# BBCG/epialleleR

Hardware: AMD Instinct MI355X
Metric: Mreads/s generateCytosineReport (150 bp PE) (higher is better)
Workload: dtype u8

## Files before the change

### epialleler_amd/csrc/common.hpp

```cpp
#pragma once
#include <hip/hip_runtime.h>
#include <stddef.h>
#include <stdint.h>
#include <string>
#include <map>
#include <memory>
#include <vector>
#include "../../include/epihip.h"

namespace epi {

void set_error(const char *fmt, ...);
int fail(int code, const char *fmt, ...);

#define EPI_HIP(expr)                                                              \
  do {                                                                             \
    hipError_t _e = (expr);                                                        \
    if (_e != hipSuccess)                                                          \
      return ::epi::fail(_e == hipErrorOutOfMemory ? EPI_ERR_NOMEM : EPI_ERR_HIP,  \
                         "%s failed: %s (%s:%d)", #expr, hipGetErrorName(_e), __FILE__, __LINE__); \
  } while (0)

#define EPI_TRY(expr) do { int _rc = (expr); if (_rc != EPI_OK) return _rc; } while (0)
constexpr int EPI_RETRY_POOL = -77;

#ifndef EPI_CX_TILE
#define EPI_CX_TILE 1024
#endif
constexpr int kTile = EPI_CX_TILE;
constexpr int kMhlTile = 512;
constexpr int kCxPlanes = 16;
constexpr int64_t kPosBias = 1LL << 31;

enum { SLOT_DOT = 0, SLOT_OTHER = 1, SLOT_H = 2, SLOT_h = 3, SLOT_X = 4, SLOT_x = 5, SLOT_Z = 6, SLOT_z = 7, SLOT_SKIP = 8 };

struct Tile {
  int64_t pos0;
  int32_t rname;
  int32_t row_lo, row_hi;
  int32_t slot;
};

struct Scalars {
  uint32_t ntiles;
  uint32_t cursor;
  uint32_t rows;
  uint32_t heavy_count;
  uint32_t deep_count;
  uint32_t fold_cursor;
  uint32_t unused6[2];
  uint32_t heavy_max;
  uint32_t unused9[3];
  uint32_t rec_max[2];
  uint32_t max_h;
  uint32_t pat_total;
};
static_assert(offsetof(Scalars, ntiles) == 0 && offsetof(Scalars, cursor) == 4 && offsetof(Scalars, rows) == 8 &&
              offsetof(Scalars, heavy_count) == 12 && offsetof(Scalars, deep_count) == 16 && offsetof(Scalars, fold_cursor) == 20 &&
              offsetof(Scalars, heavy_max) == 32 && offsetof(Scalars, rec_max) == 48 && offsetof(Scalars, max_h) == 56 &&
              offsetof(Scalars, pat_total) == 60 && sizeof(Scalars) == 64, "Scalars layout");

struct DevBuf {
  void *p = nullptr;
  size_t cap = 0;
  int ensure(size_t bytes);
  void release();
  template <class T> T *as() const { return reinterpret_cast<T *>(p); }
};

struct ProfEntry { double ms = 0; int64_t n = 0; };

struct ClassLut { uint32_t lo0, lo1, hi0, hi1; };

inline ClassLut lut16_xor_form(const ClassLut &d) {
  uint8_t D[16], L[8], H[8];
  const uint32_t w[4] = {d.lo0, d.lo1, d.hi0, d.hi1};
  for (int c = 0; c < 16; c++) D[c] = (uint8_t)(w[c >> 2] >> (8 * (c & 3)));
  auto S = [](uint8_t x) { return (uint8_t)((x & 0x80u) ? 0xFFu : 0x00u); };
  L[4] = D[4]; H[4] = D[12];
  for (int j = 5; j < 8; j++) { L[j] = (uint8_t)~D[j]; H[j] = (uint8_t)~D[8 + j]; }
  L[2] = D[2] ^ S(H[5]); L[3] = D[3] ^ S(H[7]); H[2] = D[10] ^ S(L[5]); H[3] = D[11] ^ S(L[7]);
  L[1] = D[1] ^ S(H[3]); H[1] = D[9] ^ S(L[3]);
  L[0] = D[0] ^ S(H[1]); H[0] = D[8] ^ S(L[1]);
  auto pack = [](const uint8_t *b) { return (uint32_t)b[0] | ((uint32_t)b[1] << 8) | ((uint32_t)b[2] << 16) | ((uint32_t)b[3] << 24); };
  ClassLut x;
  x.lo0 = pack(L); x.lo1 = pack(L + 4); x.hi0 = pack(H); x.hi1 = pack(H + 4);
  return x;
}
struct ThrParams {
  uint32_t min_n_ctx;
  double min_ctx_meth_frac, max_ooctx_meth_frac;
};
bool make_field_lut(const char *const cls[4], ClassLut *out);

}

struct epi_engine {
  int device = 0;
  hipStream_t stream = nullptr;
  hipStream_t copy_stream = nullptr;
  void *pinned[2] = {nullptr, nullptr};
  size_t pinned_bytes = 0;
  hipEvent_t pinned_done[2] = {nullptr, nullptr};
  hipStream_t aux_stream = nullptr;
  void *dev_stage[2] = {nullptr, nullptr};
  size_t dev_stage_bytes = 0;
  hipEvent_t up_done[2] = {nullptr, nullptr}, stage_free[2] = {nullptr, nullptr};
  int32_t *h_scalars = nullptr;
};

namespace epi {
struct RowStats {
  int32_t max_len;
  int32_t unsorted;
  int32_t bad_strand;
  int32_t bad_len;
  int32_t deep;
  uint32_t len_hist[14];
};
constexpr int kLenBinCount = 14;
constexpr int kLenBins[kLenBinCount] = {12, 16, 20, 24, 32, 40, 48, 64, 80, 96, 128, 160, 192, 0x7FFFFFFF};
}

struct epi_shard_plan;

namespace epi {
enum ReportKind {
  KIND_NONE = 0,
  KIND_CX = 1,
  KIND_MHL = 2,
  KIND_CX_SHARED = 3,
  KIND_MHL_SHARED = 4,
  KIND_MHLF_SHARED = 5,
  KIND_HET = 6,
  KIND_LINK = 7,
  KIND_HETCMP = 8,
};
}

struct epi_batch {
  epi_engine *eng = nullptr;
  int64_t n = 0, nbytes = 0;
  const uint8_t *xm = nullptr;
  const int64_t *off = nullptr;
  const int32_t *len = nullptr;
  const int32_t *rname = nullptr, *strand = nullptr, *start = nullptr;
  bool owns = false;
  int congruent = 0;
  bool cols_owned = false;
  epi::DevBuf own_xm, own_off, own_len, own_rname, own_strand, own_start;

  epi::DevBuf stats;
  bool stats_queued = false, stats_host = false;
  hipEvent_t stats_done = nullptr;
  epi::RowStats h_stats = {};
  epi::DevBuf scan_tmp;
  epi::DevBuf tiles, tile_nrow, tile_base, tile_out;
  epi::DevBuf pool_key, pool_a, pool_b, pool_c, pool_d, pool_e, pool_f;
  epi::DevBuf misc;
  epi::DevBuf mhl_m, mhl_h, mhl_blk, mhl_cont, mhl_cur;
  size_t mhl_rec_cap = 0;
  epi::DevBuf heavy_list, heavy_slab, heavy_sums;
  epi::DevBuf deep_list;
  epi::DevBuf diag;
  size_t pool_cap = 0;
  uint32_t cx_slot_cg = 0, cx_slot_wide = 0;
  uint32_t mhl_slot = 0, mhl_last_slot = 0, mhl_last_ovf = 0;
  uint32_t mhlf_slot = 0;
  bool mhlf_prefer_wide = false;
  uint32_t mhlf_prefer_wide_H = 0;
  bool mhlf_prefer_fold = false;
  epi::DevBuf mhlf_fold_slab;
  bool mhl_shared_fused = false;
  uint32_t cx_last_slot = 0, cx_last_ovf = 0;
  epi::DevBuf cx_prev_off, cx_prev_cnt;
  uint32_t cx_prev_key = 0;
  int32_t cx_prev_T = 0, cx_prev_nt = 0;
  int64_t cx_prev_nrow = 0;
  bool cx_defer = false, cx_deferred = false;
  uint32_t cx_def_heavy_done = 0;
  int32_t cx_noheavy_T = 0, cx_noheavy_rows = 0;
  int cx_last_np = 0;
  uint32_t cx_last_ctx_of_plane = 0;
  epi::DevBuf pass_tmp;
  epi::DevBuf host_io;
  epi::DevBuf bf_flag;
  int64_t patm_groups = 0, patm_pairs = 0, patm_scratch = 0;
  int64_t pats_groups = 0, pats_pairs = 0, pats_fallback = 0;
  epi::DevBuf mhl_keep_tab;
  int32_t mhl_keep_len = -1;
  double mhl_keep_oo = 0.0;
  epi::DevBuf thr_tab;
  int32_t thr_tab_len = -1;
  epi::ThrParams thr_tab_prm = {0, 0.0, 0.0};
  size_t pool_cap2 = 0;
  epi::DevBuf het_cx, het_rank, het_flag, het_key, het_sctx, het_counts, het_out, het_scal;
  int64_t het_nsite = 0, het_max_span = 0;
  int32_t het_k = 0;
  uint32_t het_min_reads = 1;
  epi::DevBuf link_back, link_blen, link_bmean, link_bflag, link_bout;
  int32_t link_D = 0;
  uint32_t link_min_reads = 1;
  int64_t link_max_dist = 0, link_nblock = 0;
  bool link_blocks = false;
  epi::DevBuf cmp_cx, cmp_counts_b;

  epi::ReportKind last_kind = epi::KIND_NONE;
  int64_t last_nrow = 0;
  int32_t last_ntiles = 0;
  int32_t tile_hint_T[4] = {0, 0, 0, 0};
  int32_t tile_hint_nt[4] = {0, 0, 0, 0};
  int32_t tile_hint_lmax[4] = {0, 0, 0, 0};
  epi::DevBuf tile_bsum[4];
  int32_t tiles_T = 0, tiles_nt = 0, tiles_lmax = 0;
  std::vector<int64_t> tiles_shared;
  epi::DevBuf tiles_nt_dev;

  std::vector<int64_t> shared_keys;
  std::vector<int32_t> shared_owned;
  std::vector<int64_t> dev_shared_keys;
  std::vector<int32_t> dev_shared_owned;
  epi::DevBuf d_shared_keys, d_shared_owned, d_slot_tile;
  int32_t *d_slab = nullptr;
  epi::DevBuf own_slab, own_slab2;
  std::vector<std::shared_ptr<epi_shard_plan>> shard_plans;
  int32_t *d_mhl_cnt_slab = nullptr;
  int64_t *d_mhl_sum_slab = nullptr;
  uint32_t mhl_ctx_mask = 0;
};

namespace epi {

hipStream_t pick_stream(epi_batch *b, void *stream);
struct CopyPart { void *dst; const void *src; size_t bytes; };
int copy_parts_to_host(epi_engine *eng, const CopyPart *parts, int nparts, hipStream_t s);
int copy_to_host(epi_engine *eng, void *h_dst, const void *d_src, size_t bytes, hipStream_t s);
int read_scalars(epi_batch *b, hipStream_t s, const void *d_src, size_t bytes, void *h_dst);
inline Scalars *report_scalars(const epi_batch *b) { return b->misc.as<Scalars>(); }
inline int read_report_scalars(epi_batch *b, hipStream_t s, Scalars *h) {
  return read_scalars(b, s, report_scalars(b), sizeof(Scalars), h);
}

void *table_block(size_t bytes);
void table_block_release(void *p);

int read_text_file(const char *path, std::vector<uint8_t> &out, int nthreads);

class BgzfWriter {
 public:
  BgzfWriter() = default;
  BgzfWriter(const BgzfWriter &) = delete;
  BgzfWriter &operator=(const BgzfWriter &) = delete;
  ~BgzfWriter();
  int open(const char *path);
  int write(const uint8_t *data, size_t n, int nthreads);
  int close();
 private:
  void *f_ = nullptr;
};

int genome_device(epi_genome *g, int device, const uint8_t **d_seq, const int64_t **d_off);

enum CallForm { CALL_XM = 0, CALL_PACKED = 1 };
struct CallRec {
  int64_t cig_off;
  int64_t seq_off;
  int64_t xm_off;
  int32_t tid, pos;
  int32_t l_seq, n_cig;
  uint8_t s_meth, s_conv;
  uint8_t pad[6];
};
static_assert(sizeof(CallRec) == 48, "CallRec layout");
struct CallWork {
  DevBuf recs, cig, seq, ref, xm;
  ~CallWork();
};
int call_methylation_window(epi_engine *eng, epi_genome *g, CallWork &wk, const CallRec *recs, int64_t nrec,
                            const uint32_t *cigar, int64_t ncig, const uint8_t *seq, int64_t nseq, int64_t nxm,
                            CallForm form, uint8_t *xm_out);

struct AsmRec {
  int64_t arena_off;
  int32_t dest0;
  int32_t n_cig, l_seq;
  int32_t pad;
};
static_assert(sizeof(AsmRec) == 24, "AsmRec layout");
struct AsmTpl {
  int64_t out_off;
  int64_t rec_lo;
  int64_t q_off;
  int32_t nrec;
  int32_t keep;
};
static_assert(sizeof(AsmTpl) == 32, "AsmTpl layout");
constexpr int kAsmLdsWidth = 2048;
int assemble_templates(epi_engine *eng, const uint8_t *d_arena, const AsmTpl *tpl, int64_t ntpl, const AsmRec *recs,
                       int64_t nrec, uint8_t q0, int32_t trim5, int64_t nbytes, int64_t qbytes, uint8_t *h_out,
                       double *t_kernel, double *t_d2h);
int stage_buffer(epi_engine *eng, int k, uint8_t **buf, size_t *cap);
int stage_send(epi_engine *eng, int k, void *d_dst, size_t bytes);

int scan_exclusive_u32(const uint32_t *d_in, uint32_t *d_out, int64_t n, uint32_t *d_total,
                       DevBuf &tmp, hipStream_t s);
int scan_block_sums_inplace(uint32_t *d_bsum, int64_t nb, uint32_t *d_total, hipStream_t s);

int launch_row_stats(epi_batch *b, hipStream_t s);
int fetch_row_stats(epi_batch *b, hipStream_t s);
int realign_batch(epi_batch *b, int modulus, hipStream_t s);
int layout_offsets(epi_batch *b, int modulus, hipStream_t s, DevBuf *new_off, unsigned long long *h_end, uint32_t *head);
int layout_group(int64_t nbytes, int64_t n);
int layout_copy_range(const uint8_t *src, int64_t c0, int64_t c1, const int64_t *src_off, const int32_t *len, const int64_t *dst_off,
                      int64_t row_a, int64_t nrows, int g, uint8_t *dst, hipStream_t s);
int build_tiles(epi_batch *b, hipStream_t s, int32_t tile_positions, RowStats *h_stats, int32_t *ntiles_out, bool *hinted = nullptr);

struct PoolLayout {
  uint32_t slot;
  size_t ovf_base;
};
int layout_pool(epi_batch *b, uint32_t slot, int T, int32_t nt, size_t headroom, int hook_slot, int (*reserve)(epi_batch *, size_t rows),
                PoolLayout *out);

struct Options {
  int device = 0;
  int cx_slot = -1;
  int cx_lean = 1;
  int cx_direct = 1;
  int heavy_rows = 0;
  int tile_hint = 1;
  int realign = 16;
  int mhl_fused = 1;
  int mhl_slot = -1;
  int mhl_wg = 0;
  int mhl_tile_group = 0;
  int mhl_multi = 0;
  int mhl_sums = 0;
  int mhlf_fold = -1;
  int mhlf_fold_slots = -1;
  int pr_group = 0;
  int pr_rpg = 0;
  int pr_wide = 1;
  int bam_timing = 0;
  int no_hugepage = 0;
  int no_libdeflate = 0;
  int pat_hash_bits = 0;
  int64_t pat_group_bytes = 0;
  int64_t upload_piece = 0;
};
const Options &options();

void prof_begin(const char *name, hipStream_t s);
void prof_end(const char *name, hipStream_t s);

#ifdef __HIPCC__
#ifdef EPI_CHECK
__device__ __forceinline__ bool epi_dev_check(uint32_t *dbg, bool ok, uint32_t code, int64_t v0, int64_t v1) {
  if (!ok && dbg && atomicCAS(dbg, 0u, code) == 0u) {
    dbg[1] = (uint32_t)v0; dbg[2] = (uint32_t)v1; dbg[3] = blockIdx.x; dbg[4] = threadIdx.x; dbg[5] = (uint32_t)(v0 >> 32);
  }
  return ok;
}
#define EPI_DEV_CHECK(dbg, ok, code, v0, v1) epi_dev_check(dbg, ok, code, v0, v1)
#else
#define EPI_DEV_CHECK(dbg, ok, code, v0, v1) true
#endif
#endif

#ifdef __HIPCC__
__device__ __forceinline__ uint32_t wave_scan_u32(uint32_t v) {
  v += (uint32_t)__builtin_amdgcn_update_dpp(0, (int)v, 0x111, 0xF, 0xF, true);
  v += (uint32_t)__builtin_amdgcn_update_dpp(0, (int)v, 0x112, 0xF, 0xF, true);
  v += (uint32_t)__builtin_amdgcn_update_dpp(0, (int)v, 0x114, 0xF, 0xF, true);
  v += (uint32_t)__builtin_amdgcn_update_dpp(0, (int)v, 0x118, 0xF, 0xF, true);
  v += (uint32_t)__builtin_amdgcn_update_dpp(0, (int)v, 0x142, 0xA, 0xF, false);
  v += (uint32_t)__builtin_amdgcn_update_dpp(0, (int)v, 0x143, 0xC, 0xF, false);
  return v;
}
__device__ __forceinline__ uint32_t wave_sum_u32(uint32_t v) {
  return (uint32_t)__builtin_amdgcn_readlane((int)wave_scan_u32(v), 63);
}
#endif

__host__ __device__ __forceinline__ uint64_t mix64(uint64_t z) {
  z += 0x9E3779B97F4A7C15ull;
  z = (z ^ (z >> 30)) * 0xBF58476D1CE4E5B9ull;
  z = (z ^ (z >> 27)) * 0x94D049BB133111EBull;
  return z ^ (z >> 31);
}
__host__ __device__ __forceinline__ uint64_t hash3(uint64_t seed, uint64_t stream, uint64_t idx) {
  return mix64(mix64(seed + stream * 0xD1B54A32D192ED03ull) ^ idx);
}

__host__ __device__ inline unsigned ctx_to_idx(unsigned char c) { return ((unsigned(c) + 2u) >> 2) & 15u; }
inline uint32_t ctx_mask_of(const char *ctx) {
  uint32_t ctx_mask = 0;
  for (const unsigned char *c = reinterpret_cast<const unsigned char *>(ctx); *c; c++) ctx_mask |= 1u << ctx_to_idx(*c);
  return ctx_mask;
}

inline int check_grid(int64_t blocks, int threads, const char *what) {
  if (blocks < 0 || blocks > 0x7FFFFFFFLL || blocks * threads >= (1LL << 32))
    return fail(EPI_ERR_ARG, "%s: batch too large for one launch (%lld workgroups of %d threads)", what, (long long)blocks, threads);
  return EPI_OK;
}


}
```

### epialleler_amd/csrc/cx_report.hip

```cpp
#include "common.hpp"
#include "tile_common.hpp"
#include <stdio.h>
#include <stdlib.h>
#include <string.h>

namespace epi {

#ifndef EPI_CX_WG
#define EPI_CX_WG 512
#endif
#ifndef EPI_CX_T1
#define EPI_CX_T1 2048
#endif
constexpr int CX_WG = EPI_CX_WG;
constexpr int CX_T1 = EPI_CX_T1;
constexpr int CX_CH = 16;
constexpr int CX_FLUSH_ROWS = 255;
constexpr int CX_SLAB_COV = 12;

struct __attribute__((packed, aligned(1))) U4u { uint32_t x, y, z, w; };

#ifndef EPI_CX_ABLATE
#define EPI_CX_ABLATE 0
#endif

struct Cx2Args {
  RowCols c;
  int64_t xm_cap;
  const Tile *tiles;
  uint32_t fill4;
  ClassLut lut_r;
  ClassLut lut_rx, lut_sx;
  ClassLut lut_s;
  ThrParams thr;
  const uint32_t *thr_tab;
  uint32_t ctx_of_plane;
  int32_t *pass_out;
  uint32_t *pool_key, *pool_meth, *pool_unmeth;
  uint32_t pool_cap;
  uint32_t *cursor;
  uint32_t slot_rows, ovf_base;
  uint32_t *tile_nrow, *tile_base;
  int32_t *slab;
  int heavy_rows;
  int heavy_chunk;
  int heavy_first;
  uint32_t *heavy_count, *heavy_max;
  uint32_t *heavy_list;
  int32_t *heavy_slab;
  uint32_t *deep_count, *deep_list;
  const uint32_t *tile_list, *tile_list_count;
  uint32_t *dbg;
  int64_t nrows;
  const uint32_t *prev_off, *prev_nrow;
  uint32_t *mismatch;
  int32_t *out[6];
  int64_t out_cap;
};

template <int T, int NP, bool LEAN = false> struct Cx2Lds {
  static constexpr int Q = T / 4;
  static constexpr int N_NARROW = 2 * NP * Q;
  static constexpr int N_CORR = 2 * Q;
  static constexpr int N_WIDE = LEAN ? 16 : 2 * NP * T;
  static constexpr int N_COV = T;
  unsigned long long *narrow, *corr;
  uint32_t *wide, *cov;
  uint32_t tid;
};

__device__ __forceinline__ uint32_t cx2_lut(uint32_t w, const ClassLut &X, uint32_t low8) {
  const uint32_t sel = (w & 0x0F0F0F0Fu) | low8;
  return __builtin_amdgcn_perm(X.lo1, X.lo0, sel) ^ __builtin_amdgcn_perm(X.hi1, X.hi0, sel ^ 0x08080808u);
}

template <int G>
__device__ __forceinline__ uint32_t cx2_group_sum(uint32_t v) {
  v += (uint32_t)__builtin_amdgcn_update_dpp(0, (int)v, 0xB1, 0xF, 0xF, true);
  v += (uint32_t)__builtin_amdgcn_update_dpp(0, (int)v, 0x4E, 0xF, 0xF, true);
  if (G >= 8) v += (uint32_t)__builtin_amdgcn_update_dpp(0, (int)v, 0x141, 0xF, 0xF, true);
  if (G >= 16) v += (uint32_t)__builtin_amdgcn_update_dpp(0, (int)v, 0x140, 0xF, 0xF, true);
  if (G >= 32) v += __shfl_xor(v, 16, 64);
  if (G >= 64) v += __shfl_xor(v, 32, 64);
  return v;
}

__device__ __forceinline__ int cx2_threshold(uint32_t n_m, uint32_t n_u, uint32_t o_m, uint32_t o_u, const ThrParams &prm) {
  int res = 0;
  if (n_m != 0) {
    const unsigned n_all = n_m + n_u;
    if (!(n_all < prm.min_n_ctx)) {
      const double frac = (double)n_m / (double)n_all;
      if (!(frac < prm.min_ctx_meth_frac)) {
        res = 1;
        if (o_m > 0) {
          const unsigned o_all = o_m + o_u;
          const double ofrac = (double)o_m / (double)o_all;
          if (ofrac > prm.max_ooctx_meth_frac) res = 0;
        }
      }
    }
  }
  return res;
}

__device__ __forceinline__ int cx2_threshold_tab(uint32_t n_m, uint32_t n_u, uint32_t o_m, uint32_t o_u, const ThrParams &prm,
                                                 const uint32_t *__restrict__ tab) {
  const uint32_t n_all = n_m + n_u, o_all = o_m + o_u;
  const uint32_t least = tab[n_all] & 0xFFFFu, most = tab[o_all] >> 16;
  return n_m != 0u && !(n_all < prm.min_n_ctx) && n_m >= least && (o_m == 0u || o_m <= most);
}

__global__ __launch_bounds__(256) void k_thr_table(ThrParams prm, int32_t nmax, uint32_t *__restrict__ tab) {
  const int32_t n = (int32_t)(blockIdx.x * 256 + threadIdx.x);
  if (n > nmax) return;
  uint32_t least = 0xFFFFu, most = 0u;
  if (n >= 1) {
    int32_t lo = 1, hi = n + 1;
    while (lo < hi) {
      const int32_t m = (lo + hi) >> 1;
      const double frac = (double)(uint32_t)m / (double)(uint32_t)n;
      if (!(frac < prm.min_ctx_meth_frac)) hi = m; else lo = m + 1;
    }
    if (lo <= n) least = (uint32_t)lo;
    lo = 1; hi = n + 1;
    while (lo < hi) {
      const int32_t m = (lo + hi) >> 1;
      const double frac = (double)(uint32_t)m / (double)(uint32_t)n;
      if (frac > prm.max_ooctx_meth_frac) hi = m; else lo = m + 1;
    }
    most = (uint32_t)(lo - 1);
  }
  tab[n] = least | (most << 16);
}

struct Cx2Row {
  const uint8_t *base;
  int32_t rel, len;
  int32_t c0, clast;
  bool edge;
  int sidx, ps;
};

__device__ __forceinline__ void cx2_mask_from(int lo , uint32_t (&m)[4]) {
  const unsigned long long x = ~0ull << ((8 * lo) & 63);
  const bool low = lo < 8;
  const unsigned long long a = low ? x : 0ull, b = low ? ~0ull : x;
  m[0] = (uint32_t)a; m[1] = (uint32_t)(a >> 32); m[2] = (uint32_t)b; m[3] = (uint32_t)(b >> 32);
}
__device__ __forceinline__ void cx2_mask_upto(int hi , uint32_t (&m)[4]) {
  const int sh = 8 * (16 - hi);
  const unsigned long long x = ~0ull >> (sh & 63);
  const bool high = sh < 64;
  const unsigned long long a = high ? ~0ull : x, b = high ? x : 0ull;
  m[0] = (uint32_t)a; m[1] = (uint32_t)(a >> 32); m[2] = (uint32_t)b; m[3] = (uint32_t)(b >> 32);
}

template <int T, int G, int NU, int NP, bool FUSED, int MODE = 0, class LT, class F>
__device__ __forceinline__ void cx2_visit(const Cx2Args &a, Cx2Row &g, int32_t cs, int32_t cz, int sub, int rcur,
                                          const LT &L, F fetch_next, uint32_t *carry = nullptr) {
  constexpr int C = T / CX_CH, Q = LT::Q;
  const int32_t cb = cs + sub;
  const int32_t tl = cz - cb;
  uint32_t w[NU][4];
  if (__builtin_expect(g.edge, 0)) {
#pragma unroll
    for (int u = 0; u < NU; u++) {
#pragma unroll
      for (int d = 0; d < 4; d++) {
        uint32_t x = a.fill4;
        if (u * G <= tl) {
          const int64_t ad = (g.base - a.c.xm) + CX_CH * (int64_t)(cb + u * G) + 4 * d;
          x = 0;
#pragma unroll
          for (int j = 0; j < 4; j++) {
            const int64_t q = ad + j;
            const uint32_t byte = (q >= 0 && q < a.xm_cap) ? (uint32_t)a.c.xm[q] : (a.fill4 & 255u);
            x |= byte << (8 * j);
          }
        }
        w[u][d] = x;
      }
    }
  } else {
    const uint8_t *p = g.base + CX_CH * (int64_t)cb;
    {
      const int32_t uq = tl / G < NU - 1 ? tl / G : NU - 1;
      const int64_t a_lo = p - a.c.xm, a_hi = a_lo + (tl >= 0 ? CX_CH * (int64_t)(uq * G) + CX_CH : 0);
      (void)a_lo; (void)a_hi;
      if (!EPI_DEV_CHECK(a.dbg, tl < 0 || (a_lo >= 0 && a_hi <= a.xm_cap), 21, a_lo, a_hi)) return;
    }
    if (EPI_CX_ABLATE & 1) p = reinterpret_cast<const uint8_t *>(reinterpret_cast<uintptr_t>(p) & ~(uintptr_t)15);
#pragma unroll
    for (int u = 0; u < NU; u++) {
      if (u * G <= tl) {
        const U4u v = *reinterpret_cast<const U4u *>(p + CX_CH * u * G);
        w[u][0] = v.x; w[u][1] = v.y; w[u][2] = v.z; w[u][3] = v.w;
      } else {
        w[u][0] = w[u][1] = w[u][2] = w[u][3] = a.fill4;
      }
    }
  }
  fetch_next();
  if (EPI_CX_ABLATE & 8) {
    uint32_t x = 0;
#pragma unroll
    for (int u = 0; u < NU; u++) x ^= w[u][0] ^ w[u][1] ^ w[u][2] ^ w[u][3];
    if (x == 0x12345678u) atomicAdd(L.cov, 1u);
    return;
  }
  {
    uint32_t mf[4], ml[4];
    cx2_mask_from(cb == g.c0 ? (g.rel & 15) : 0, mf);
    cx2_mask_upto(((g.rel + g.len - 1) & 15) + 1, ml);
#pragma unroll
    for (int d = 0; d < 4; d++) { asm("" : "+v"(mf[d])); asm("" : "+v"(ml[d])); }
#pragma unroll
    for (int d = 0; d < 4; d++) w[0][d] = (w[0][d] & mf[d]) | (a.fill4 & ~mf[d]);
#pragma unroll
    for (int u = 0; u < NU; u++) {
      const bool last = cb + u * G == g.clast;
      if (__ballot(last) != 0ull) {
        const uint32_t keep = last ? 0u : 0xFFFFFFFFu;
#pragma unroll
        for (int d = 0; d < 4; d++) {
          const uint32_t m = ml[d] | keep;
          w[u][d] = (w[u][d] & m) | (a.fill4 & ~m);
        }
      }
    }
  }

  unsigned long long *nar = L.narrow + g.sidx * NP * Q + 4 * cb;
  unsigned long long *cor = L.corr + g.sidx * Q + 4 * cb;
  if constexpr (FUSED) {
    static_assert(NP == 1, "fused thresholding: one reported context, the thresholding context");
    uint32_t cls[4] = {0, 0, 0, 0}, fl = 0;
#pragma unroll
    for (int u = 0; u < NU; u++) {
#pragma unroll
      for (int d = 0; d < 4; d++) w[u][d] = (EPI_CX_ABLATE & 4) ? w[u][d] : cx2_lut(w[u][d], a.lut_sx, 0u);
      fl |= w[u][0] | w[u][1] | w[u][2] | w[u][3];
    }
    auto count = [&](auto masked) {
      constexpr bool MASKED = decltype(masked)::value;
      constexpr uint32_t EV = MASKED ? 0x55555555u : 0xFFFFFFFFu;
      uint32_t E = 0, O = 0;
#pragma unroll
      for (int u = 0; u < NU; u++) {
        const uint32_t t = (w[u][0] & EV) + (w[u][1] & EV) + (w[u][2] & EV);
        const uint32_t d3 = w[u][3] & EV;
        E += (t & 0x33333333u) + (d3 & 0x33333333u);
        O += ((t >> 2) & 0x33333333u) + ((d3 >> 2) & 0x33333333u);
        if (u % 3 == 2 || u == NU - 1) {
          cls[0] = __builtin_amdgcn_sad_u8(E & 0x0F0F0F0Fu, 0u, cls[0]);
          cls[2] = __builtin_amdgcn_sad_u8((E >> 4) & 0x0F0F0F0Fu, 0u, cls[2]);
          cls[1] = __builtin_amdgcn_sad_u8(O & 0x0F0F0F0Fu, 0u, cls[1]);
          cls[3] = __builtin_amdgcn_sad_u8((O >> 4) & 0x0F0F0F0Fu, 0u, cls[3]);
          E = 0; O = 0;
        }
      }
    };
    if constexpr (MODE != 2) {
      if (__builtin_expect(__ballot((fl & 0xAAAAAAAAu) != 0u) == 0ull, 1)) count(std::false_type{});
      else count(std::true_type{});
    }
    if constexpr (MODE == 1) {
#pragma unroll
      for (int k = 0; k < 4; k++) carry[k] += cls[k];
      return;
    }
    if constexpr (MODE == 0) {
      const uint32_t s01 = cx2_group_sum<G>(cls[0] | (cls[1] << 16)), s23 = cx2_group_sum<G>(cls[2] | (cls[3] << 16));
      const uint32_t n_all = s01 & 0xFFFFu, n_m = s01 >> 16;
      g.ps = a.thr_tab ? cx2_threshold_tab(n_m, n_all - n_m, s23 & 0xFFFFu, s23 >> 16, a.thr, a.thr_tab)
                       : cx2_threshold(n_m, n_all - n_m, s23 & 0xFFFFu, s23 >> 16, a.thr);
      if (a.pass_out && sub == 0 && (uint32_t)g.rel < (uint32_t)T) a.pass_out[rcur] = g.ps;
    }
    const uint32_t pm = g.ps ? 0x01010101u : 0u;
#pragma unroll
    for (int u = 0; u < NU; u++) {
      const bool inside = (uint32_t)(cb + u * G) < (uint32_t)C;
#pragma unroll
      for (int d = 0; d < 4; d++) {
        const uint32_t lo = w[u][d] & 0x01010101u, hi = (w[u][d] >> 2) & pm;
        if (lo != 0u && inside && !(EPI_CX_ABLATE & 2)) atomicAdd(nar + 4 * u * G + d, (unsigned long long)lo | ((unsigned long long)hi << 32));
      }
    }
    const uint32_t fsel = g.ps ? 0x0A0A0A0Au : 0xA0A0A0A0u;
    if (__builtin_expect((fl & fsel) != 0u, 0)) {
      const int sh = g.ps ? 1 : 5;
#pragma unroll
      for (int u = 0; u < NU; u++) {
        const bool inside = (uint32_t)(cb + u * G) < (uint32_t)C;
#pragma unroll
        for (int d = 0; d < 4; d++) {
          const uint32_t sk = (w[u][d] >> sh) & 0x01010101u, db = (w[u][d] >> (sh + 2)) & 0x01010101u;
          if ((sk | db) != 0u && inside) atomicAdd(cor + 4 * u * G + d, (unsigned long long)sk | ((unsigned long long)db << 32));
        }
      }
    }
  } else if constexpr (NP == 1 && G >= 16) {
    const bool passing = g.ps != 0;
    const uint32_t k77 = (a.ctx_of_plane & 255u) * 0x11111111u;
    const uint32_t rm = passing ? 0xDDDDDDDDu : 0x55555555u, rv = passing ? 0x99999999u : 0x11111111u;
    uint32_t clean = 0xFFFFFFFFu;
#pragma unroll
    for (int u = 0; u < NU; u++) {
      const bool inside = (uint32_t)(cb + u * G) < (uint32_t)C;
#pragma unroll
      for (int e = 0; e < 2; e++) {
        const uint32_t pk = (w[u][2 * e] & 0x0F0F0F0Fu) | ((w[u][2 * e + 1] << 4) & 0xF0F0F0F0u);
        const uint32_t z = ((pk & 0x77777777u) ^ k77) + 0x77777777u;
        const uint32_t np = ~z & 0x88888888u;
        const uint32_t t = (pk & rm) ^ rv;
        clean &= ((t & 0x77777777u) + 0x77777777u) | t;
        if (np != 0u && inside && !(EPI_CX_ABLATE & 2)) {
          const uint32_t up = passing ? np & ~pk : 0u;
          const uint32_t n0 = (np >> 3) & 0x01010101u, n1 = (np >> 7) & 0x01010101u;
          if (n0 != 0u) atomicAdd(nar + 4 * u * G + 2 * e, (unsigned long long)n0 | ((unsigned long long)((up >> 3) & 0x01010101u) << 32));
          if (n1 != 0u) atomicAdd(nar + 4 * u * G + 2 * e + 1, (unsigned long long)n1 | ((unsigned long long)((up >> 7) & 0x01010101u) << 32));
        }
      }
    }
    if (__builtin_expect((~clean & 0x88888888u) != 0u, 0)) {
      const uint32_t pick0 = passing ? 0u : 0x08080808u;
#pragma unroll
      for (int u = 0; u < NU; u++) {
        const bool inside = (uint32_t)(cb + u * G) < (uint32_t)C;
#pragma unroll
        for (int d = 0; d < 4; d++) {
          const uint32_t f = cx2_lut(w[u][d], a.lut_rx, pick0);
          const uint32_t sk = (f >> 6) & 0x01010101u, db = (f >> 7) & 0x01010101u;
          if ((sk | db) != 0u && inside) atomicAdd(cor + 4 * u * G + d, (unsigned long long)sk | ((unsigned long long)db << 32));
        }
      }
    }
  } else {
    const uint32_t pick0 = g.ps == 0 ? 0x08080808u : 0u;
    uint32_t fl = 0;
#pragma unroll
    for (int u = 0; u < NU; u++) {
      const bool inside = (uint32_t)(cb + u * G) < (uint32_t)C;
#pragma unroll
      for (int d = 0; d < 4; d++) {
        const uint32_t f = cx2_lut(w[u][d], a.lut_rx, pick0);
        w[u][d] = f;
        fl |= f;
#pragma unroll
        for (int p = 0; p < NP; p++) {
          const uint32_t lo = (f >> (2 * p)) & 0x01010101u, hi = (f >> (2 * p + 1)) & 0x01010101u;
          if (lo != 0u && inside && !(EPI_CX_ABLATE & 2))
            atomicAdd(nar + p * Q + 4 * u * G + d, (unsigned long long)lo | ((unsigned long long)hi << 32));
        }
      }
    }
    if (__builtin_expect((fl & 0xC0C0C0C0u) != 0u, 0)) {
#pragma unroll
      for (int u = 0; u < NU; u++) {
        const bool inside = (uint32_t)(cb + u * G) < (uint32_t)C;
#pragma unroll
        for (int d = 0; d < 4; d++) {
          const uint32_t sk = (w[u][d] >> 6) & 0x01010101u, db = (w[u][d] >> 7) & 0x01010101u;
          if ((sk | db) != 0u && inside) atomicAdd(cor + 4 * u * G + d, (unsigned long long)sk | ((unsigned long long)db << 32));
        }
      }
    }
  }
}

template <int T, int G, int NU, int NP, bool FUSED, int WG, class LT>
__device__ __forceinline__ void cx2_rows(const Cx2Args &a, const Tile &td, int row_lo, int row_hi, const LT &L) {
  constexpr int R = 64 / G, NW = WG / 64, C = T / CX_CH;
  const int lane = L.tid & 63, wave = L.tid >> 6;
  const int sub = lane & (G - 1), grp = lane / G;
  Tile tb = td;
  tb.row_hi = row_hi;
  int r = row_lo + wave * R + grp;
  RowVals v = cx_load_row(a.c, tb, r);
  for (int rbase = row_lo + wave * R; rbase < row_hi; rbase += NW * R) {
    const int rcur = r;
    if (!EPI_DEV_CHECK(a.dbg, !v.ok || (rcur >= 0 && rcur < a.nrows && v.len >= 0 && (v.sd == 1 || v.sd == 2 || v.len == 0)), 22, rcur, v.sd)) return;
    r += NW * R;
    RowVals nv;
    bool fetched = false;
    auto fetch_next = [&]() { if (!fetched) { nv = cx_load_row(a.c, tb, r); fetched = true; } };
    if (v.ok && v.len > 0 && (int32_t)((uint32_t)v.st - (uint32_t)td.pos0) + v.len > 0) {
      Cx2Row g;
      g.rel = (int32_t)((uint32_t)v.st - (uint32_t)td.pos0);
      g.len = v.len;
      g.c0 = g.rel >> 4;
      g.clast = (g.rel + v.len - 1) >> 4;
      g.base = a.c.xm + (v.o - g.rel);
      g.edge = v.o < CX_CH || v.o + v.len + CX_CH > a.xm_cap;
      g.sidx = v.sd - 1;
      g.ps = v.ps;
      if constexpr (FUSED) {
        if (__builtin_expect(__ballot(g.clast - g.c0 >= G * NU) == 0ull, 1)) {
          cx2_visit<T, G, NU, NP, true>(a, g, g.c0, g.clast, sub, rcur, L, fetch_next);
        } else {
          uint32_t cls[4] = {0, 0, 0, 0};
          for (int32_t cs = g.c0; __ballot(cs <= g.clast) != 0ull; cs += G * NU)
            cx2_visit<T, G, NU, NP, true, 1>(a, g, cs, g.clast, sub, rcur, L, fetch_next, cls);
          const uint32_t s01 = cx2_group_sum<G>(cls[0] | (cls[1] << 16)), s23 = cx2_group_sum<G>(cls[2] | (cls[3] << 16));
          const uint32_t n_all = s01 & 0xFFFFu, n_m = s01 >> 16;
          g.ps = a.thr_tab ? cx2_threshold_tab(n_m, n_all - n_m, s23 & 0xFFFFu, s23 >> 16, a.thr, a.thr_tab)
                           : cx2_threshold(n_m, n_all - n_m, s23 & 0xFFFFu, s23 >> 16, a.thr);
          if (a.pass_out && sub == 0 && (uint32_t)g.rel < (uint32_t)T) a.pass_out[rcur] = g.ps;
          const int32_t ca = g.c0 > 0 ? g.c0 : 0, cz = g.clast < C - 1 ? g.clast : C - 1;
          for (int32_t cs = ca; __ballot(cs <= cz) != 0ull; cs += G * NU)
            cx2_visit<T, G, NU, NP, true, 2>(a, g, cs, cz, sub, rcur, L, fetch_next);
        }
      } else {
        const int32_t ca = g.c0 > 0 ? g.c0 : 0, cz = g.clast < C - 1 ? g.clast : C - 1;
        if (__builtin_expect(__ballot(cz - ca >= G * NU) == 0ull, 1)) {
          cx2_visit<T, G, NU, NP, false>(a, g, ca, cz, sub, rcur, L, fetch_next);
        } else {
          for (int32_t cs = ca; __ballot(cs <= cz) != 0ull; cs += G * NU) cx2_visit<T, G, NU, NP, false>(a, g, cs, cz, sub, rcur, L, fetch_next);
        }
      }
      if (sub == 0) {
        const int32_t ca = g.rel > 0 ? g.rel : 0, cb = g.rel + v.len < T ? g.rel + v.len : T;
        const uint32_t unit = g.sidx ? 65536u : 1u;
        if (ca < cb && !(EPI_CX_ABLATE & 32)) { atomicAdd(L.cov + ca, unit); if (cb < T) atomicAdd(L.cov + cb, 0u - unit); }
      }
    } else if (FUSED && v.ok && sub == 0 && a.pass_out && (uint32_t)((uint32_t)v.st - (uint32_t)td.pos0) < (uint32_t)T) {
      a.pass_out[rcur] = 0;
    }
    fetch_next();
    v = nv;
  }
}

template <int T, int NP, bool LEAN, int WG>
__device__ __forceinline__ void cx2_flush(const Cx2Lds<T, NP, LEAN> &L) {
  constexpr int Q = Cx2Lds<T, NP, LEAN>::Q;
  if constexpr (!LEAN) {
    for (int i = L.tid; i < 2 * NP * Q; i += WG) {
      const unsigned long long v = L.narrow[i];
      if (v == 0ull) continue;
      L.narrow[i] = 0ull;
      const uint32_t lo = (uint32_t)v, hi = (uint32_t)(v >> 32);
      const int sp = i / Q, q = i - sp * Q;
      uint4 *wd = reinterpret_cast<uint4 *>(L.wide + sp * T + 4 * q);
      uint4 c = *wd;
      c.x += (lo & 255u) | ((hi & 255u) << 16);
      c.y += ((lo >> 8) & 255u) | (((hi >> 8) & 255u) << 16);
      c.z += ((lo >> 16) & 255u) | (((hi >> 16) & 255u) << 16);
      c.w += (lo >> 24) | ((hi >> 24) << 16);
      *wd = c;
    }
  }
  for (int i = L.tid; i < 2 * Q; i += WG) {
    const unsigned long long v = L.corr[i];
    if (v == 0ull) continue;
    L.corr[i] = 0ull;
    const uint32_t sk = (uint32_t)v, db = (uint32_t)(v >> 32);
    const int s = i / Q, q = i - s * Q;
    const int32_t unit = s ? 65536 : 1;
    int32_t prev = 0;
#pragma unroll
    for (int j = 0; j < 4; j++) {
      const int32_t d = (int32_t)((db >> (8 * j)) & 255u) - (int32_t)((sk >> (8 * j)) & 255u);
      if (d != prev) atomicAdd(L.cov + 4 * q + j, (uint32_t)((d - prev) * unit));
      prev = d;
    }
    if (prev != 0 && 4 * q + 4 < T) atomicAdd(L.cov + 4 * q + 4, (uint32_t)(-prev * unit));
  }
}

__device__ __forceinline__ uint32_t cx_pool_reserve(const Cx2Args &a, int tile, uint32_t n, bool *fits) {
  if (n <= a.slot_rows) { *fits = true; return (uint32_t)tile * a.slot_rows; }
  const uint32_t o = atomicAdd(a.cursor, n);
  *fits = (uint64_t)a.ovf_base + o + n <= a.pool_cap;
  return a.ovf_base + o;
}

__device__ __forceinline__ void cx_direct_none(const Cx2Args &a, int tile, uint32_t tid = threadIdx.x) {
  if (a.prev_off && tid == 0 && a.prev_nrow[tile] != 0u) atomicAdd(a.mismatch, 1u);
}

template <int T, int NP> struct CxSrcLds {
  const uint32_t *wide, *cov;
  __device__ __forceinline__ uint32_t any(int sd, int pos) const {
    uint32_t x = 0;
#pragma unroll
    for (int p = 0; p < NP; p++) x |= wide[(sd * NP + p) * T + pos];
    return x;
  }
  __device__ __forceinline__ void pair(int sd, int p, int pos, uint32_t *n, uint32_t *M) const {
    const uint32_t w = wide[(sd * NP + p) * T + pos];
    *n = w & 0xFFFFu; *M = w >> 16;
  }
  __device__ __forceinline__ uint32_t coverage(int sd, int pos) const { const uint32_t v = cov[pos]; return sd ? v >> 16 : v & 0xFFFFu; }
};
template <int QS> struct CxSrcU8 {
  const uint32_t *narrow;
  const uint32_t *cov;
  __device__ __forceinline__ uint32_t any(int sd, int pos) const {
    return (narrow[2 * (sd * QS + (pos >> 2))] >> (8 * (pos & 3))) & 255u;
  }
  __device__ __forceinline__ void pair(int sd, int, int pos, uint32_t *n, uint32_t *M) const {
    const uint2 c = *reinterpret_cast<const uint2 *>(narrow + 2 * (sd * QS + (pos >> 2)));
    *n = (c.x >> (8 * (pos & 3))) & 255u; *M = (c.y >> (8 * (pos & 3))) & 255u;
  }
  __device__ __forceinline__ uint32_t coverage(int sd, int pos) const { const uint32_t v = cov[pos]; return sd ? v >> 16 : v & 0xFFFFu; }
};
template <int T, int NP> struct CxSrcSlab {
  const int32_t *slab;
  const uint32_t *cov;
  __device__ __forceinline__ uint32_t any(int sd, int pos) const {
    uint32_t x = 0;
#pragma unroll
    for (int p = 0; p < NP; p++) x |= (uint32_t)slab[(2 * (sd * NP + p)) * T + pos];
    return x;
  }
  __device__ __forceinline__ void pair(int sd, int p, int pos, uint32_t *n, uint32_t *M) const {
    *n = (uint32_t)slab[(2 * (sd * NP + p)) * T + pos]; *M = (uint32_t)slab[(2 * (sd * NP + p) + 1) * T + pos];
  }
  __device__ __forceinline__ uint32_t coverage(int sd, int pos) const { return cov[sd * T + pos]; }
};

template <int T, int WG = CX_WG>
__device__ __forceinline__ void cx2_prefix(uint32_t *arr, uint32_t *s_scan, uint32_t tid = threadIdx.x) {
  constexpr int PPT = T / WG, NW = WG / 64;
  static_assert(PPT >= 1 && PPT <= 8, "prefix layout");
  const int lane = tid & 63, wave = tid >> 6;
  uint32_t x[PPT];
#pragma unroll
  for (int j = 0; j < PPT; j++) x[j] = arr[tid * PPT + j];
#pragma unroll
  for (int j = 1; j < PPT; j++) x[j] += x[j - 1];
  const uint32_t inc = wave_scan_u32(x[PPT - 1]);
  if (lane == 63) s_scan[wave] = inc;
  __syncthreads();
  uint32_t before = inc - x[PPT - 1];
#pragma unroll
  for (int w = 0; w < NW; w++) before += w < wave ? s_scan[w] : 0u;
#pragma unroll
  for (int j = 0; j < PPT; j++) arr[tid * PPT + j] = x[j] + before;
  __syncthreads();
}

template <int T, int NP, int WG = CX_WG, class SRC>
__device__ __forceinline__ void cx2_emit(const Cx2Args &a, int tile, const SRC &src, uint32_t *s_scan, uint16_t *s_list, uint32_t tid = threadIdx.x) {
  constexpr int NW = WG / 64, PW = T / NW, IT = PW / 32;
  static_assert(PW % 32 == 0 && IT >= 1 && IT <= 16, "emit phase layout");
  const int lane = tid & 63, wave = tid >> 6;
  const int l5 = lane & 31, sd = lane >> 5;
  const uint32_t below = (1u << l5) - 1u;
  uint16_t *list = s_list + wave * (2 * PW);
  uint32_t nc = 0;
#pragma unroll
  for (int i = 0; i < IT; i++) {
    const uint32_t any = src.any(sd, wave * PW + i * 32 + l5);
    const unsigned long long bal = __ballot(any != 0u);
    const uint32_t blo = (uint32_t)bal, bhi = (uint32_t)(bal >> 32);
    const uint32_t rank = (uint32_t)__popc(blo & below) + (uint32_t)__popc(bhi & below) + (sd ? (blo >> l5) & 1u : 0u);
    if (any != 0u) list[nc + rank] = (uint16_t)(i * 64 + lane);
    nc += (uint32_t)__popcll(bal);
  }
  uint32_t key[IT], me[IT], un[IT], off[IT];
  bool ok[IT];
  uint32_t carry = 0;
#pragma unroll
  for (int jj = 0; jj < IT; jj++) {
    ok[jj] = false; key[jj] = 0; me[jj] = 0; un[jj] = 0; off[jj] = 0;
    if ((uint32_t)(jj * 64) < nc) {
      const uint32_t j = (uint32_t)(jj * 64 + lane);
      bool good = false;
      if (j < nc) {
        const uint32_t id = list[j];
        const int pos = wave * PW + (int)(id >> 6) * 32 + (int)(id & 31u), st = (int)((id >> 5) & 1u);
        const uint32_t half = src.coverage(st, pos) >> 1;
        uint32_t ctx = 0, m = 0, u = 0;
#pragma unroll
        for (int p = 0; p < NP; p++) {
          uint32_t nn, M;
          src.pair(st, p, pos, &nn, &M);
          if (nn > half && ctx == 0) { ctx = (a.ctx_of_plane >> (8 * p)) & 255u; m = M; u = nn - M; }
        }
        good = ctx != 0;
        key[jj] = ((uint32_t)pos << 4) | ((uint32_t)st << 3) | ctx;
        me[jj] = m;
        un[jj] = u;
      }
      const unsigned long long be = __ballot(good);
      off[jj] = carry + __builtin_amdgcn_mbcnt_hi((uint32_t)(be >> 32), __builtin_amdgcn_mbcnt_lo((uint32_t)be, 0u));
      carry += (uint32_t)__popcll(be);
      ok[jj] = good;
    }
  }
  if (lane == 0) s_scan[wave] = carry;
  __syncthreads();
  if (a.prev_off) {
    if (tid == 0) {
      uint32_t acc = 0;
      for (int w = 0; w < NW; w++) { const uint32_t t = s_scan[w]; s_scan[w] = acc; acc += t; }
      const uint32_t base = a.prev_off[tile];
      const bool good = acc == a.prev_nrow[tile] && (int64_t)base + acc <= a.out_cap;
      if (!good) atomicAdd(a.mismatch, 1u);
      s_scan[NW + 1] = good ? base : 0xFFFFFFFFu;
    }
    __syncthreads();
    const uint32_t base = s_scan[NW + 1];
    if (base != 0xFFFFFFFFu) {
      const Tile td = a.tiles[tile];
      const uint32_t w0 = base + s_scan[wave];
#pragma unroll
      for (int jj = 0; jj < IT; jj++) {
        if (ok[jj]) {
          const uint32_t o = w0 + off[jj];
          a.out[0][o] = td.rname;
          a.out[1][o] = 1 + (int32_t)((key[jj] >> 3) & 1u);
          a.out[2][o] = (int32_t)(td.pos0 + (int64_t)(key[jj] >> 4));
          a.out[3][o] = (int32_t)(key[jj] & 7u);
          a.out[4][o] = (int32_t)me[jj];
          a.out[5][o] = (int32_t)un[jj];
        }
      }
    }
    return;
  }
  if (tid == 0) {
    uint32_t acc = 0;
    for (int w = 0; w < NW; w++) { const uint32_t t = s_scan[w]; s_scan[w] = acc; acc += t; }
    s_scan[NW] = acc;
    uint32_t base = 0;
    bool fits = true;
    if (acc) base = cx_pool_reserve(a, tile, acc, &fits);
    s_scan[NW + 1] = base;
    s_scan[NW] = fits ? acc : 0xFFFFFFFFu;
    a.tile_nrow[tile] = acc;
    a.tile_base[tile] = base;
  }
  __syncthreads();
  const uint32_t total = s_scan[NW], base = s_scan[NW + 1];
  if (total != 0xFFFFFFFFu) {
    const uint32_t w0 = base + s_scan[wave];
#pragma unroll
    for (int jj = 0; jj < IT; jj++) {
      if (ok[jj]) {
        const uint32_t w = w0 + off[jj];
        if (!EPI_DEV_CHECK(a.dbg, w < a.pool_cap, 23, w, a.pool_cap)) continue;
        a.pool_key[w] = key[jj];
        a.pool_meth[w] = me[jj];
        a.pool_unmeth[w] = un[jj];
      }
    }
  }
}

template <int T, int NP, bool LEAN, int WG>
__device__ __forceinline__ void cx2_dump_slab(const Cx2Lds<T, NP, LEAN> &L, int32_t *slab) {
  uint32_t *dst = reinterpret_cast<uint32_t *>(slab);
  if constexpr (LEAN) {
    constexpr int Q = Cx2Lds<T, NP, LEAN>::Q;
    for (int i = L.tid; i < 2 * NP * Q; i += WG) {
      const unsigned long long v = L.narrow[i];
      if (v == 0ull) continue;
      const uint32_t lo = (uint32_t)v, hi = (uint32_t)(v >> 32);
      const int sp = i / Q, q = i - sp * Q;
#pragma unroll
      for (int j = 0; j < 4; j++) {
        const uint32_t n = (lo >> (8 * j)) & 255u, M = (hi >> (8 * j)) & 255u;
        if (n) atomicAdd(dst + (2 * sp) * T + 4 * q + j, n);
        if (M) atomicAdd(dst + (2 * sp + 1) * T + 4 * q + j, M);
      }
    }
  } else {
    for (int i = L.tid; i < 2 * NP * T; i += WG) {
      const uint32_t v = L.wide[i];
      if (!v) continue;
      const int sp = i / T, p = i - sp * T;
      if (v & 0xFFFFu) atomicAdd(dst + (2 * sp) * T + p, v & 0xFFFFu);
      if (v >> 16) atomicAdd(dst + (2 * sp + 1) * T + p, v >> 16);
    }
  }
  for (int p = L.tid; p < T; p += WG) {
    const uint32_t v = L.cov[p];
    if (!v) continue;
    const int32_t lo = (int32_t)(int16_t)(v & 0xFFFFu);
    const int32_t hi = ((int32_t)v - lo) >> 16;
    if (lo) atomicAdd(dst + CX_SLAB_COV * T + p, (uint32_t)lo);
    if (hi) atomicAdd(dst + (CX_SLAB_COV + 1) * T + p, (uint32_t)hi);
  }
}

__device__ __forceinline__ int cx_tile_of_block(int b, int ntiles) {
  const int chunk = (ntiles + 7) >> 3;
  return (b & 7) * chunk + (b >> 3);
}

template <int T, int NP, bool LEAN = false> constexpr int cx2_lds_bytes() {
  using LdsT = Cx2Lds<T, NP, LEAN>;
  return (LdsT::N_NARROW + LdsT::N_CORR) * 8 + (LdsT::N_WIDE + LdsT::N_COV) * 4;
}
#ifndef EPI_CX_WPS
#define EPI_CX_WPS 8
#endif
template <int T, int NP, int NU = 3, bool LEAN = false, int WG = CX_WG> constexpr int cx2_waves_per_simd() {
  const int by_lds = (160 * 1024) / (cx2_lds_bytes<T, NP, LEAN>() + 64), by_thr = 2048 / WG;
  int wgs = by_lds < by_thr ? by_lds : by_thr;
  if (NU >= 4 && wgs * WG > 1536) wgs = 1536 / WG;
  if (wgs * WG / 256 > EPI_CX_WPS) wgs = EPI_CX_WPS * 256 / WG;
  return (wgs < 1 ? 1 : wgs) * WG / 256;
}

#define CX2_SHARED(T, NP, LEAN)                                                                                  \
  using LdsT = Cx2Lds<T, NP, LEAN>;                                                                              \
  __shared__ __attribute__((aligned(16))) unsigned long long s_u8[LdsT::N_NARROW + LdsT::N_CORR];                \
  __shared__ __attribute__((aligned(16))) uint32_t s_wide[LdsT::N_WIDE];                                         \
  __shared__ __attribute__((aligned(16))) uint32_t s_cov[LdsT::N_COV];                                           \
  static_assert((LdsT::N_NARROW + LdsT::N_CORR) * 8 >= 4 * T + 64 && LdsT::N_CORR * 8 >= 4 * T, "the candidate lists and the scan scratch reuse dead arrays"); \
  uint32_t *s_scan = LEAN ? s_wide : reinterpret_cast<uint32_t *>(s_u8) + T;                                      \
  uint16_t *s_list = reinterpret_cast<uint16_t *>(LEAN ? s_u8 + LdsT::N_NARROW : s_u8);                          \
  (void)s_scan; (void)s_list;                                                                                     \
  LdsT L;                                                                                                         \
  L.narrow = s_u8; L.corr = s_u8 + LdsT::N_NARROW; L.wide = s_wide; L.cov = s_cov; L.tid = threadIdx.x;

template <int T, int NP, bool LEAN, int WG>
__device__ __forceinline__ void cx2_clear(const Cx2Lds<T, NP, LEAN> &L) {
  using LdsT = Cx2Lds<T, NP, LEAN>;
  uint4 *z = reinterpret_cast<uint4 *>(L.narrow);
  for (int i = L.tid; i < (LdsT::N_NARROW + LdsT::N_CORR) / 2; i += WG) z[i] = make_uint4(0, 0, 0, 0);
  if constexpr (!LEAN) {
    uint4 *y = reinterpret_cast<uint4 *>(L.wide);
    for (int i = L.tid; i < LdsT::N_WIDE / 4; i += WG) y[i] = make_uint4(0, 0, 0, 0);
  }
  uint4 *x = reinterpret_cast<uint4 *>(L.cov);
  for (int i = L.tid; i < LdsT::N_COV / 4; i += WG) x[i] = make_uint4(0, 0, 0, 0);
}

template <int T, int G, int NU, int NP, bool FUSED, bool LEAN, int WG>
__device__ __forceinline__ void cx2_accumulate(const Cx2Args &a, const Tile &td, int row_lo, int row_hi, const Cx2Lds<T, NP, LEAN> &L) {
  if constexpr (LEAN) {
    cx2_rows<T, G, NU, NP, FUSED, WG>(a, td, row_lo, row_hi, L);
  } else {
    for (int b0 = row_lo; b0 < row_hi; b0 += CX_FLUSH_ROWS) {
      if (b0 > row_lo) { __syncthreads(); cx2_flush<T, NP, LEAN, WG>(L); __syncthreads(); }
      cx2_rows<T, G, NU, NP, FUSED, WG>(a, td, b0, b0 + CX_FLUSH_ROWS < row_hi ? b0 + CX_FLUSH_ROWS : row_hi, L);
    }
  }
  __syncthreads();
  cx2_flush<T, NP, LEAN, WG>(L);
  __syncthreads();
}

#ifndef EPI_CX_LEAN_WG
#define EPI_CX_LEAN_WG 256
#endif
template <bool LEAN> constexpr int cx2_wg() { return LEAN ? EPI_CX_LEAN_WG : CX_WG; }

template <int T, int G, int NU, int NP, bool FUSED, bool LEAN, class LdsT>
__device__ __forceinline__ void cx2_tile(const Cx2Args &a, int tile, const Tile &td, const LdsT &L, uint32_t *s_scan, uint16_t *s_list, int *s_flag) {
  constexpr int WG = cx2_wg<LEAN>();
  cx2_clear<T, NP, LEAN, WG>(L);
  if (td.row_hi - td.row_lo > a.heavy_rows) {
    if (L.tid == 0) {
      const uint32_t h = atomicAdd(a.heavy_count, 1u);
      a.heavy_list[h] = (uint32_t)tile;
      atomicMax(a.heavy_max, (uint32_t)(td.row_hi - td.row_lo));
      a.tile_nrow[tile] = 0;
      a.tile_base[tile] = 0;
    }
    cx_direct_none(a, tile, L.tid);
    return;
  }
  if constexpr (LEAN) {
    if (a.deep_list && td.row_hi - td.row_lo > CX_FLUSH_ROWS) {
      if (L.tid == 0) *s_flag = 0;
      __syncthreads();
      bool deep = false;
      for (int x = td.row_lo + (int)L.tid; x + CX_FLUSH_ROWS < td.row_hi; x += WG)
        deep |= (int64_t)a.c.start[x + CX_FLUSH_ROWS] < (int64_t)a.c.start[x] + a.c.len[x];
      if (deep) *s_flag = 1;
      __syncthreads();
      if (*s_flag) {
        if (L.tid == 0) { a.deep_list[atomicAdd(a.deep_count, 1u)] = (uint32_t)tile; a.tile_nrow[tile] = 0; a.tile_base[tile] = 0; }
        cx_direct_none(a, tile, L.tid);
        return;
      }
    }
  }
  __syncthreads();
  cx2_accumulate<T, G, NU, NP, FUSED, LEAN, WG>(a, td, td.row_lo, td.row_hi, L);
  if (td.slot >= 0) {
    cx2_dump_slab<T, NP, LEAN, WG>(L, a.slab + (int64_t)td.slot * (kCxPlanes * T));
    if (L.tid == 0) { a.tile_nrow[tile] = 0; a.tile_base[tile] = 0; }
    cx_direct_none(a, tile, L.tid);
    return;
  }
  if (EPI_CX_ABLATE & 16) { if (L.tid == 0) { a.tile_nrow[tile] = 0; a.tile_base[tile] = 0; } cx_direct_none(a, tile, L.tid); return; }
  cx2_prefix<T, WG>(L.cov, s_scan, L.tid);
  if constexpr (LEAN) {
    static_assert(NP == 1, "the u8 counters serve single-context reports");
    CxSrcU8<LdsT::Q> src;
    src.narrow = reinterpret_cast<const uint32_t *>(L.narrow); src.cov = L.cov;
    cx2_emit<T, NP, WG>(a, tile, src, s_scan, s_list, L.tid);
  } else {
    CxSrcLds<T, NP> src;
    src.wide = L.wide; src.cov = L.cov;
    cx2_emit<T, NP, WG>(a, tile, src, s_scan, s_list, L.tid);
  }
}

template <int T, int G, int NU, int NP, bool FUSED, bool LEAN>
__global__ __launch_bounds__(cx2_wg<LEAN>(), (cx2_waves_per_simd<T, NP, NU, LEAN, cx2_wg<LEAN>()>())) void k_cx_tiles(Cx2Args a, int ntiles) {
  CX2_SHARED(T, NP, LEAN)
  __shared__ int s_flag;
  if constexpr (!LEAN) {
    if (a.tile_list) {
      const uint32_t n = *a.tile_list_count;
      for (uint32_t i = blockIdx.x; i < n; i += gridDim.x) {
        const int tile = (int)a.tile_list[i];
        const Tile td = a.tiles[tile];
        cx2_tile<T, G, NU, NP, FUSED, LEAN>(a, tile, td, L, s_scan, s_list, &s_flag);
        __syncthreads();
      }
      return;
    }
  }
  const int tile = cx_tile_of_block(blockIdx.x, ntiles);
  if (tile >= ntiles) return;
  const Tile td = a.tiles[tile];
  cx2_tile<T, G, NU, NP, FUSED, LEAN>(a, tile, td, L, s_scan, s_list, &s_flag);
}

template <int T, int G, int NU, int NP, bool FUSED>
__global__ __launch_bounds__(CX_WG, (cx2_waves_per_simd<T, NP, NU>())) void k_cx_heavy(Cx2Args a) {
  CX2_SHARED(T, NP, false)
  const uint32_t hi_idx = (uint32_t)a.heavy_first + blockIdx.y;
  if (hi_idx >= *a.heavy_count) return;
  const int tile = (int)a.heavy_list[hi_idx];
  const Tile td = a.tiles[tile];
  for (int lo = td.row_lo + (int)blockIdx.x * a.heavy_chunk; lo < td.row_hi; lo += (int)gridDim.x * a.heavy_chunk) {
    const int hi = td.row_hi - lo > a.heavy_chunk ? lo + a.heavy_chunk : td.row_hi;
    cx2_clear<T, NP, false, CX_WG>(L);
    __syncthreads();
    cx2_accumulate<T, G, NU, NP, FUSED, false, CX_WG>(a, td, lo, hi, L);
    cx2_dump_slab<T, NP, false, CX_WG>(L, td.slot >= 0 ? a.slab + (int64_t)td.slot * (kCxPlanes * T)
                                          : a.heavy_slab + (int64_t)blockIdx.y * (kCxPlanes * T));
    __syncthreads();
  }
}

template <int T, int NP>
__device__ __forceinline__ void cx2_emit_from_slab(const Cx2Args &a, int tile, const int32_t *slab) {
  __shared__ __attribute__((aligned(16))) uint32_t s_cov[2 * T];
  __shared__ uint32_t s_scan[CX_WG / 64 + 2];
  __shared__ uint16_t s_list[2 * T];
  for (int i = threadIdx.x; i < 2 * T; i += CX_WG) s_cov[i] = (uint32_t)slab[CX_SLAB_COV * T + i];
  __syncthreads();
  cx2_prefix<T>(s_cov, s_scan);
  cx2_prefix<T>(s_cov + T, s_scan);
  CxSrcSlab<T, NP> src;
  src.slab = slab; src.cov = s_cov;
  cx2_emit<T, NP>(a, tile, src, s_scan, s_list);
}

template <int T, int NP>
__global__ __launch_bounds__(CX_WG) void k_cx_emit_heavy(Cx2Args a) {
  const uint32_t hi_idx = (uint32_t)a.heavy_first + blockIdx.x;
  if (hi_idx >= *a.heavy_count) return;
  const int tile = (int)a.heavy_list[hi_idx];
  if (a.tiles[tile].slot >= 0) return;
  cx2_emit_from_slab<T, NP>(a, tile, a.heavy_slab + (int64_t)blockIdx.x * (kCxPlanes * T));
}

template <int T, int NP>
__global__ __launch_bounds__(CX_WG) void k_cx_emit_slab(Cx2Args a, const int32_t *__restrict__ owned,
                                                         const int32_t *__restrict__ slot_tile) {
  if (!owned[blockIdx.x]) return;
  const int tile = slot_tile[blockIdx.x];
  if (tile < 0) return;
  cx2_emit_from_slab<T, NP>(a, tile, a.slab + (int64_t)a.tiles[tile].slot * (kCxPlanes * T));
}

#ifndef EPI_CXP_T
#define EPI_CXP_T 1024
#endif
constexpr int CXP_T = EPI_CXP_T;

template <int G, int U0, int U1>
__device__ __forceinline__ void cxp_add_range(const uint32_t (&w)[CX_NU], const RowSlice &cur) {
  if constexpr (U0 < U1) {
    if (U0 * G <= cur.tl) cx_add_dword<CXP_T, 4 * G * U0, U0 == 0>(w[U0], cur.tl == U0 * G, cur);
    cxp_add_range<G, U0 + 1, U1>(w, cur);
  }
}

template <int G>
__device__ __forceinline__ void cxp_accumulate(const RowCols &c, const Tile &td, uint32_t *cnt) {
  constexpr int R = 64 / G, NW = CX_WG / 64;
  const int lane = threadIdx.x & 63, wave = threadIdx.x >> 6;
  const int sub = lane & (G - 1), grp = lane / G;
  int r = td.row_lo + wave * R + grp;
  RowSlice cur = cx_row_slice<CXP_T, G>(c, td, r, sub, cnt);
  for (int rbase = td.row_lo + wave * R; rbase < td.row_hi; rbase += NW * R) {
    uint32_t w[CX_NU];
#pragma unroll
    for (int u = 0; u < CX_NU; u++) w[u] = u * G <= cur.tl ? cur.src[u * G] : 0u;
    r += NW * R;
    const RowSlice nxt = cx_row_slice<CXP_T, G>(c, td, r, sub, cnt);
    cxp_add_range<G, 0, CX_NU>(w, cur);
    for (int k = sub + CX_NU * G; k < cur.nd; k += G) {
      RowSlice t = cur;
#pragma unroll
      for (int j = 0; j < 4; j++) t.dst[j] = cur.dst[j] + 4 * (k - sub);
      cx_add_dword<CXP_T, 0, false>(cur.src[k - sub], k == cur.nd - 1, t);
    }
    cur = nxt;
  }
}

__device__ __forceinline__ void cxp_convert(uint32_t *cnt) {
  constexpr int T = CXP_T;
  for (int i = threadIdx.x; i < 2 * T; i += CX_WG) {
    uint32_t *c0 = cnt + (i / T) * 4 * T + (i % T);
    const uint32_t d0 = c0[0], dh = c0[T], dx = c0[2 * T], dz = c0[3 * T];
    const uint32_t nh = (dh & 0xFFFFu) + (dh >> 16), nx = (dx & 0xFFFFu) + (dx >> 16), nz = (dz & 0xFFFFu) + (dz >> 16);
    c0[0] = (d0 & 0xFFFFu) + (d0 >> 16) + nh + nx + nz;
    c0[T] = nh | (dh << 16);
    c0[2 * T] = nx | (dx << 16);
    c0[3 * T] = nz | (dz << 16);
  }
}

struct CxSrcPk {
  const uint32_t *cnt;
  int pl[3];
  __device__ __forceinline__ uint32_t any(int sd, int pos) const {
    uint32_t x = 0;
#pragma unroll
    for (int p = 0; p < 3; p++) if (pl[p]) x |= cnt[(sd * 4 + pl[p]) * CXP_T + pos];
    return x;
  }
  __device__ __forceinline__ void pair(int sd, int p, int pos, uint32_t *n, uint32_t *M) const {
    const uint32_t w = pl[p] ? cnt[(sd * 4 + pl[p]) * CXP_T + pos] : 0u;
    *n = w & 0xFFFFu; *M = w >> 16;
  }
  __device__ __forceinline__ uint32_t coverage(int sd, int pos) const { return cnt[sd * 4 * CXP_T + pos]; }
};

__device__ __forceinline__ CxSrcPk cxp_source(const Cx2Args &a, const uint32_t *cnt) {
  CxSrcPk s;
  s.cnt = cnt;
#pragma unroll
  for (int p = 0; p < 3; p++) { const uint32_t k = (a.ctx_of_plane >> (8 * p)) & 255u; s.pl[p] = k == 2u ? 1 : k == 6u ? 2 : k == 7u ? 3 : 0; }
  return s;
}

__device__ __forceinline__ void cxp_dump_slab(const Cx2Args &a, const uint32_t *cnt, int np, int32_t *slab) {
  constexpr int T = CXP_T;
  uint32_t *dst = reinterpret_cast<uint32_t *>(slab);
  const CxSrcPk src = cxp_source(a, cnt);
  for (int i = threadIdx.x; i < 2 * T; i += CX_WG) {
    const int sd = i / T, pos = i % T;
#pragma unroll
    for (int p = 0; p < 3; p++) {
      if (p >= np) break;
      uint32_t n, M;
      src.pair(sd, p, pos, &n, &M);
      if (n) atomicAdd(dst + (2 * (sd * np + p)) * T + pos, n);
      if (M) atomicAdd(dst + (2 * (sd * np + p) + 1) * T + pos, M);
    }
    const uint32_t d = src.coverage(sd, pos) - (pos ? src.coverage(sd, pos - 1) : 0u);
    if (d) atomicAdd(dst + (CX_SLAB_COV + sd) * T + pos, d);
  }
}

#define CXP_SHARED                                                                                      \
  __shared__ __attribute__((aligned(16))) uint32_t cnt_raw[8 * CXP_T + 2 * kCxGuard];                  \
  __shared__ uint32_t s_scan[CX_WG / 64 + 2];                                                         \
  __shared__ uint16_t s_list[2 * CXP_T];                                                               \
  uint32_t *cnt = cnt_raw + kCxGuard;

template <int G>
__global__ __launch_bounds__(CX_WG, 8) void k_cxp_tiles(Cx2Args a, int ntiles, int np) {
  CXP_SHARED
  const int tile = cx_tile_of_block(blockIdx.x, ntiles);
  if (tile >= ntiles) return;
  const Tile td = a.tiles[tile];
  uint4 *z = reinterpret_cast<uint4 *>(cnt_raw);
  for (int i = threadIdx.x; i < (8 * CXP_T + 2 * kCxGuard) / 4; i += CX_WG) z[i] = make_uint4(0, 0, 0, 0);
  if (td.row_hi - td.row_lo > a.heavy_rows) {
    if (threadIdx.x == 0) {
      const uint32_t h = atomicAdd(a.heavy_count, 1u);
      a.heavy_list[h] = (uint32_t)tile;
      atomicMax(a.heavy_max, (uint32_t)(td.row_hi - td.row_lo));
      a.tile_nrow[tile] = 0;
      a.tile_base[tile] = 0;
    }
    cx_direct_none(a, tile);
    return;
  }
  __syncthreads();
  cxp_accumulate<G>(a.c, td, cnt);
  __syncthreads();
  cxp_convert(cnt);
  __syncthreads();
  if (td.slot >= 0) {
    cxp_dump_slab(a, cnt, np, a.slab + (int64_t)td.slot * (kCxPlanes * CXP_T));
    if (threadIdx.x == 0) { a.tile_nrow[tile] = 0; a.tile_base[tile] = 0; }
    cx_direct_none(a, tile);
    return;
  }
  if (EPI_CX_ABLATE & 16) {
    if (threadIdx.x == 0) { a.tile_nrow[tile] = 0; a.tile_base[tile] = 0; }
    cx_direct_none(a, tile);
    return;
  }
  cx2_emit<CXP_T, 3>(a, tile, cxp_source(a, cnt), s_scan, s_list);
}

template <int G>
__global__ __launch_bounds__(CX_WG, 8) void k_cxp_heavy(Cx2Args a, int np) {
  CXP_SHARED
  (void)s_scan; (void)s_list;
  const uint32_t hi_idx = (uint32_t)a.heavy_first + blockIdx.y;
  if (hi_idx >= *a.heavy_count) return;
  const int tile = (int)a.heavy_list[hi_idx];
  const Tile whole = a.tiles[tile];
  for (int lo = whole.row_lo + (int)blockIdx.x * a.heavy_chunk; lo < whole.row_hi; lo += (int)gridDim.x * a.heavy_chunk) {
    Tile td = whole;
    td.row_lo = lo;
    if (td.row_hi - lo > a.heavy_chunk) td.row_hi = lo + a.heavy_chunk;
    uint4 *z = reinterpret_cast<uint4 *>(cnt_raw);
    for (int i = threadIdx.x; i < (8 * CXP_T + 2 * kCxGuard) / 4; i += CX_WG) z[i] = make_uint4(0, 0, 0, 0);
    __syncthreads();
    cxp_accumulate<G>(a.c, td, cnt);
    __syncthreads();
    cxp_convert(cnt);
    __syncthreads();
    cxp_dump_slab(a, cnt, np, td.slot >= 0 ? a.slab + (int64_t)td.slot * (kCxPlanes * CXP_T)
                                            : a.heavy_slab + (int64_t)blockIdx.y * (kCxPlanes * CXP_T));
    __syncthreads();
  }
}

struct __attribute__((packed, aligned(4))) CxU4u { uint32_t x, y, z, w; };

__global__ __launch_bounds__(256) void k_cx_gather(const Tile *__restrict__ tiles, const uint32_t *__restrict__ tile_out,
                                                    const uint32_t *__restrict__ tile_nrow, const uint32_t *__restrict__ tile_base,
                                                    int32_t ntiles, const uint32_t *__restrict__ pool_key,
                                                    const uint32_t *__restrict__ pool_meth, const uint32_t *__restrict__ pool_unmeth,
                                                    int32_t *__restrict__ o_rname, int32_t *__restrict__ o_strand,
                                                    int32_t *__restrict__ o_pos, int32_t *__restrict__ o_ctx,
                                                    int32_t *__restrict__ o_meth, int32_t *__restrict__ o_unmeth) {
  const int tile = blockIdx.x * 4 + (threadIdx.x >> 6);
  if (tile >= ntiles) return;
  const uint32_t n = tile_nrow[tile];
  if (n == 0) return;
  const int lane = threadIdx.x & 63;
  const Tile td = tiles[tile];
  const uint32_t src0 = tile_base[tile], dst0 = tile_out[tile];
  const uint32_t n4 = n & ~3u;
  for (uint32_t i = 4u * lane; i < n4; i += 256) {
    const CxU4u key = *reinterpret_cast<const CxU4u *>(pool_key + src0 + i);
    const CxU4u me = *reinterpret_cast<const CxU4u *>(pool_meth + src0 + i);
    const CxU4u un = *reinterpret_cast<const CxU4u *>(pool_unmeth + src0 + i);
    const uint32_t o = dst0 + i;
    const uint32_t rn = (uint32_t)td.rname;
    const uint32_t p0 = (uint32_t)td.pos0;
    *reinterpret_cast<CxU4u *>(o_rname + o) = CxU4u{rn, rn, rn, rn};
    *reinterpret_cast<CxU4u *>(o_strand + o) = CxU4u{1u + ((key.x >> 3) & 1u), 1u + ((key.y >> 3) & 1u), 1u + ((key.z >> 3) & 1u), 1u + ((key.w >> 3) & 1u)};
    *reinterpret_cast<CxU4u *>(o_pos + o) = CxU4u{p0 + (key.x >> 4), p0 + (key.y >> 4), p0 + (key.z >> 4), p0 + (key.w >> 4)};
    *reinterpret_cast<CxU4u *>(o_ctx + o) = CxU4u{key.x & 7u, key.y & 7u, key.z & 7u, key.w & 7u};
    *reinterpret_cast<CxU4u *>(o_meth + o) = me;
    *reinterpret_cast<CxU4u *>(o_unmeth + o) = un;
  }
  for (uint32_t i = n4 + lane; i < n; i += 64) {
    const uint32_t key = pool_key[src0 + i];
    const uint32_t o = dst0 + i;
    o_rname[o] = td.rname;
    o_strand[o] = 1 + (int32_t)((key >> 3) & 1u);
    o_pos[o] = (int32_t)(td.pos0 + (int64_t)(key >> 4));
    o_ctx[o] = (int32_t)(key & 7u);
    o_meth[o] = (int32_t)pool_meth[src0 + i];
    o_unmeth[o] = (int32_t)pool_unmeth[src0 + i];
  }
}


static int cx_tile_for(int np) { return np <= 1 ? CX_T1 : CXP_T; }

static int pick_cx_shape(const RowStats &st, int T, bool fused, bool lean) {
#ifdef EPI_CX_FORCE_SHAPE
  if (fused) return EPI_CX_FORCE_SHAPE;
#endif
  const int max_chunks = (int)(((int64_t)st.max_len + 2 * (CX_CH - 1)) / CX_CH);
  const int tile_chunks = T / CX_CH;
  double total = 0;
  for (int k = 0; k < kLenBinCount; k++) total += st.len_hist[k];
  int best = 64 * 8 + 3;
  double best_cost = -1;
  for (int g = (fused || lean) ? 4 : 8; g <= 64; g <<= 1)
    for (int nu = 3; nu <= (lean ? 6 : 3); nu++) {
      const int cap = g * nu;
      double extra = 0;
      for (int k = 0; k < kLenBinCount; k++) {
        if (!st.len_hist[k]) continue;
        int ch = kLenBins[k] < max_chunks ? kLenBins[k] : max_chunks;
        if (!fused && ch > tile_chunks) ch = tile_chunks;
        const int slices = (ch + cap - 1) / cap;
        if (slices > 1) extra += (total > 0 ? st.len_hist[k] / total : 1.0) * (fused ? 2 * slices - 1 : slices - 1);
      }
      if (total == 0) {
        int ch = max_chunks;
        if (!fused && ch > tile_chunks) ch = tile_chunks;
        if (cap < ch) continue;
      }
      const double cost = (cap + 2.0 * g) * (1.0 + (64 / g) * extra);
      if (best_cost < 0 || cost < best_cost) { best = g * 8 + nu; best_cost = cost; }
    }
  return best;
}
static bool cx_fused_fits(const RowStats &st) {
  if (st.max_len >= 65000) return false;
  double total = 0, longer = 0;
  for (int k = 0; k < kLenBinCount; k++) { total += st.len_hist[k]; if (kLenBins[k] > 64 * 3) longer += st.len_hist[k]; }
  if (total == 0) return ((int64_t)st.max_len + 2 * (CX_CH - 1)) / CX_CH <= 64 * 3;
  return longer <= 0.01 * total;
}

constexpr unsigned CX_HEAVY_CAP = 8, CX_HEAVY_GRID = 128;
constexpr unsigned CX_LIST_GRID = 512;

template <int T, int NU, int NP, bool FUSED, bool LEAN>
static void launch_cx_tiles(int g, int nt, hipStream_t s, const Cx2Args &a) {
  const unsigned nb = a.tile_list ? CX_LIST_GRID : (unsigned)(((nt + 7) / 8) * 8);
  switch (g) {
    case 4: if constexpr (FUSED || LEAN) { hipLaunchKernelGGL((k_cx_tiles<T, 4, NU, NP, FUSED, LEAN>), dim3(nb), dim3(cx2_wg<LEAN>()), 0, s, a, nt); } break;
    case 8: hipLaunchKernelGGL((k_cx_tiles<T, 8, NU, NP, FUSED, LEAN>), dim3(nb), dim3(cx2_wg<LEAN>()), 0, s, a, nt); break;
    case 16: hipLaunchKernelGGL((k_cx_tiles<T, 16, NU, NP, FUSED, LEAN>), dim3(nb), dim3(cx2_wg<LEAN>()), 0, s, a, nt); break;
    case 32: hipLaunchKernelGGL((k_cx_tiles<T, 32, NU, NP, FUSED, LEAN>), dim3(nb), dim3(cx2_wg<LEAN>()), 0, s, a, nt); break;
    default: hipLaunchKernelGGL((k_cx_tiles<T, 64, NU, NP, FUSED, LEAN>), dim3(nb), dim3(cx2_wg<LEAN>()), 0, s, a, nt); break;
  }
}

template <int T, int NU, int NP, bool FUSED>
static void launch_cx_g(bool heavy, bool lean, int g, int nt, dim3 grid, hipStream_t s, const Cx2Args &a) {
  if (!heavy) {
    if (lean) launch_cx_tiles<T, NU, NP, FUSED, true>(g, nt, s, a);
    else launch_cx_tiles<T, NU, NP, FUSED, false>(g, nt, s, a);
    return;
  }
  switch (g) {
    case 4: if constexpr (FUSED) { hipLaunchKernelGGL((k_cx_heavy<T, 4, NU, NP, FUSED>), grid, dim3(CX_WG), 0, s, a); } break;
    case 8: hipLaunchKernelGGL((k_cx_heavy<T, 8, NU, NP, FUSED>), grid, dim3(CX_WG), 0, s, a); break;
    case 16: hipLaunchKernelGGL((k_cx_heavy<T, 16, NU, NP, FUSED>), grid, dim3(CX_WG), 0, s, a); break;
    case 32: hipLaunchKernelGGL((k_cx_heavy<T, 32, NU, NP, FUSED>), grid, dim3(CX_WG), 0, s, a); break;
    default: hipLaunchKernelGGL((k_cx_heavy<T, 64, NU, NP, FUSED>), grid, dim3(CX_WG), 0, s, a); break;
  }
  hipLaunchKernelGGL((k_cx_emit_heavy<T, NP>), dim3(grid.y), dim3(CX_WG), 0, s, a);
}

static int pick_cxp_group(int32_t max_len) {
  const int slice = (max_len < CXP_T ? max_len : CXP_T) + 3;
  const int nd = (slice + 3) / 4;
  int g = 8;
  while (g < 64 && g * CX_NU < nd) g <<= 1;
  return g;
}
static int pick_cxp_group(const RowStats &st) {
  const int by_max = pick_cxp_group(st.max_len);
  double total = 0;
  for (int k = 0; k < kLenBinCount; k++) total += st.len_hist[k];
  if (total == 0) return by_max;
  for (int g = 8; g < by_max; g <<= 1) {
    double longer = 0;
    for (int k = 0; k < kLenBinCount; k++) {
      const int64_t len_k = (int64_t)kLenBins[k] * 16 - 15;
      const int64_t slice = (len_k < CXP_T ? len_k : CXP_T) + 3;
      if ((slice + 3) / 4 > (int64_t)g * CX_NU) longer += st.len_hist[k];
    }
    if (longer <= 0.005 * total) return g;
  }
  return by_max;
}

static void launch_cxp(bool heavy, int np, int g, int nt, dim3 grid, hipStream_t s, const Cx2Args &a) {
  if (!heavy) {
    const unsigned nb = (unsigned)(((nt + 7) / 8) * 8);
    switch (g) {
      case 8: hipLaunchKernelGGL((k_cxp_tiles<8>), dim3(nb), dim3(CX_WG), 0, s, a, nt, np); break;
      case 16: hipLaunchKernelGGL((k_cxp_tiles<16>), dim3(nb), dim3(CX_WG), 0, s, a, nt, np); break;
      case 32: hipLaunchKernelGGL((k_cxp_tiles<32>), dim3(nb), dim3(CX_WG), 0, s, a, nt, np); break;
      default: hipLaunchKernelGGL((k_cxp_tiles<64>), dim3(nb), dim3(CX_WG), 0, s, a, nt, np); break;
    }
    return;
  }
  switch (g) {
    case 8: hipLaunchKernelGGL((k_cxp_heavy<8>), grid, dim3(CX_WG), 0, s, a, np); break;
    case 16: hipLaunchKernelGGL((k_cxp_heavy<16>), grid, dim3(CX_WG), 0, s, a, np); break;
    case 32: hipLaunchKernelGGL((k_cxp_heavy<32>), grid, dim3(CX_WG), 0, s, a, np); break;
    default: hipLaunchKernelGGL((k_cxp_heavy<64>), grid, dim3(CX_WG), 0, s, a, np); break;
  }
  if (np == 2) hipLaunchKernelGGL((k_cx_emit_heavy<CXP_T, 2>), dim3(grid.y), dim3(CX_WG), 0, s, a);
  else hipLaunchKernelGGL((k_cx_emit_heavy<CXP_T, 3>), dim3(grid.y), dim3(CX_WG), 0, s, a);
}

static void launch_cx(bool heavy, int np, bool fused, bool lean, int shape, int nt, dim3 grid, hipStream_t s, const Cx2Args &a) {
  const int g = shape >> 3;
  if (np > 1) { launch_cxp(heavy, np, g, nt, grid, s, a); return; }
  if (!heavy && lean && (shape & 7) > 3) {
    switch (shape & 7) {
      case 4: if (fused) launch_cx_tiles<CX_T1, 4, 1, true, true>(g, nt, s, a); else launch_cx_tiles<CX_T1, 4, 1, false, true>(g, nt, s, a); break;
      case 5: if (fused) launch_cx_tiles<CX_T1, 5, 1, true, true>(g, nt, s, a); else launch_cx_tiles<CX_T1, 5, 1, false, true>(g, nt, s, a); break;
      default: if (fused) launch_cx_tiles<CX_T1, 6, 1, true, true>(g, nt, s, a); else launch_cx_tiles<CX_T1, 6, 1, false, true>(g, nt, s, a); break;
    }
    return;
  }
  if (fused) launch_cx_g<CX_T1, 3, 1, true>(heavy, lean, g, nt, grid, s, a);
  else launch_cx_g<CX_T1, 3, 1, false>(heavy, lean, g, nt, grid, s, a);
}

static void launch_cx_emit_slab(int np, int nshared, hipStream_t s, const Cx2Args &a, const int32_t *owned, const int32_t *slot_tile) {
  if (np == 1) hipLaunchKernelGGL((k_cx_emit_slab<CX_T1, 1>), dim3((unsigned)nshared), dim3(CX_WG), 0, s, a, owned, slot_tile);
  else if (np == 2) hipLaunchKernelGGL((k_cx_emit_slab<CXP_T, 2>), dim3((unsigned)nshared), dim3(CX_WG), 0, s, a, owned, slot_tile);
  else hipLaunchKernelGGL((k_cx_emit_slab<CXP_T, 3>), dim3((unsigned)nshared), dim3(CX_WG), 0, s, a, owned, slot_tile);
}

static int ensure_pool(epi_batch *b, size_t rows) {
  if (rows <= b->pool_cap && b->pool_key.p) return EPI_OK;
  EPI_TRY(b->pool_key.ensure(rows * 4));
  EPI_TRY(b->pool_a.ensure(rows * 4));
  EPI_TRY(b->pool_b.ensure(rows * 4));
  b->pool_cap = rows;
  return EPI_OK;
}

static int make_report_lut(uint32_t ctx_mask, ClassLut *lut, uint32_t *ctx_of_plane) {
  uint32_t f[16] = {0};
  int np = 0;
  *ctx_of_plane = 0;
  for (uint32_t k : {2u, 6u, 7u}) {
    if (!((ctx_mask >> k) & 1u)) continue;
    f[k] |= 3u << (2 * np);
    f[k + 8] |= 1u << (2 * np);
    *ctx_of_plane |= k << (8 * np);
    np++;
  }
  f[11] |= 0x40u;
  f[9] |= 0x80u;
  auto pack = [&](int b0) { return f[b0] | (f[b0 + 1] << 8) | (f[b0 + 2] << 16) | (f[b0 + 3] << 24); };
  lut->lo0 = pack(0); lut->lo1 = pack(4); lut->hi0 = pack(8); lut->hi1 = pack(12);
  return np;
}

static uint32_t lut_byte(const ClassLut &l, int code) {
  const uint32_t w = code < 4 ? l.lo0 : code < 8 ? l.lo1 : code < 12 ? l.hi0 : l.hi1;
  return (w >> (8 * (code & 3))) & 255u;
}

struct CxThreshold {
  const char *cls[4];
  ThrParams prm;
};

static bool make_fused_lut(const CxThreshold &t, uint32_t ctx_of_plane, int np, ClassLut *lut, uint32_t *fill4) {
  if (np != 1) return false;
  const uint32_t k = ctx_of_plane & 255u;
  unsigned w[4][16] = {{0}};
  for (int c = 0; c < 4; c++)
    if (t.cls[c]) for (const unsigned char *p = reinterpret_cast<const unsigned char *>(t.cls[c]); *p; p++) w[c][ctx_to_idx(*p)]++;
  for (int c = 0; c < 4; c++) for (int i = 0; i < 16; i++) if (w[c][i] > 1) return false;
  for (uint32_t i = 0; i < 16; i++) {
    if ((w[0][i] != 0) != (i == k)) return false;
    if ((w[1][i] != 0) != (i == (k | 8u))) return false;
  }
  uint32_t f[16];
  for (uint32_t i = 0; i < 16; i++) {
    f[i] = 0;
    if (i == k || i == (k | 8u)) f[i] |= 0x01u;
    if (i == k) f[i] |= 0x04u;
    if (w[2][i]) f[i] |= 0x10u;
    if (w[3][i]) f[i] |= 0x40u;
    if (i == 11) f[i] |= 0x02u;
    if (i == 9) f[i] |= 0x08u;
    if ((i | 8u) == 11) f[i] |= 0x20u;
    if ((i | 8u) == 9) f[i] |= 0x80u;
  }
  int fill = -1;
  for (int c : {12, 8, 0, 4}) if (f[c] == 0) { fill = c; break; }
  if (fill < 0) return false;
  auto pack = [&](int b0) { return f[b0] | (f[b0 + 1] << 8) | (f[b0 + 2] << 16) | (f[b0 + 3] << 24); };
  lut->lo0 = pack(0); lut->lo1 = pack(4); lut->hi0 = pack(8); lut->hi1 = pack(12);
  *fill4 = 0x01010101u * (uint32_t)fill;
  return true;
}

static int64_t cx_recorded_nrow(const epi_batch *b, uint32_t ctx_mask) {
  return b->cx_prev_key == (ctx_mask | 0x80000000u) ? b->cx_prev_nrow : -1;
}

struct CxPlan {
  int T, np;
  int32_t nt;
  bool nt_hinted;
  bool fused;
  bool lean;
  bool per_tile;
  bool chained;
  int shape, shape_heavy;
  int32_t nshared;
  size_t headroom;
  PoolLayout pool;
};

static int cx_check_tile_count(epi_batch *b, bool hinted, uint32_t counted, int32_t nt) {
  if (!hinted || counted == (uint32_t)nt) return EPI_OK;
  for (int i = 0; i < 4; i++) b->tile_hint_T[i] = 0;
  return fail(EPI_ERR_STATE, "the rows of this batch changed since an earlier report (tile count %u, was %d)", counted, nt);
}

static int cx_setup_threshold(epi_batch *b, const CxThreshold &thr, const RowStats &st, CxPlan &p, int32_t *d_pass_out, hipStream_t s,
                              Cx2Args &a, const int32_t **d_pass) {
  uint32_t fill4 = 0;
  if (p.nt > 0 && p.np > 0 && cx_fused_fits(st) && make_fused_lut(thr, a.ctx_of_plane, p.np, &a.lut_s, &fill4)) {
    p.fused = true;
    a.lut_sx = lut16_xor_form(a.lut_s);
    a.thr = thr.prm;
    a.fill4 = fill4;
    a.pass_out = d_pass_out;
    const bool same = b->thr_tab_len == st.max_len && b->thr_tab_prm.min_n_ctx == thr.prm.min_n_ctx &&
                      memcmp(&b->thr_tab_prm.min_ctx_meth_frac, &thr.prm.min_ctx_meth_frac, sizeof(double)) == 0 &&
                      memcmp(&b->thr_tab_prm.max_ooctx_meth_frac, &thr.prm.max_ooctx_meth_frac, sizeof(double)) == 0;
    if (!same) {
      EPI_TRY(b->thr_tab.ensure((size_t)(st.max_len + 1) * 4));
      hipLaunchKernelGGL(k_thr_table, dim3((unsigned)(st.max_len / 256 + 1)), dim3(256), 0, s, thr.prm, st.max_len, b->thr_tab.as<uint32_t>());
      EPI_HIP(hipGetLastError());
      b->thr_tab_len = st.max_len;
      memset(&b->thr_tab_prm, 0, sizeof(ThrParams));
      b->thr_tab_prm.min_n_ctx = thr.prm.min_n_ctx;
      b->thr_tab_prm.min_ctx_meth_frac = thr.prm.min_ctx_meth_frac;
      b->thr_tab_prm.max_ooctx_meth_frac = thr.prm.max_ooctx_meth_frac;
    }
    a.thr_tab = b->thr_tab.as<uint32_t>();
  } else if (b->n > 0) {
    int32_t *dst = d_pass_out;
    if (!dst) { EPI_TRY(b->pass_tmp.ensure((size_t)b->n * 4)); dst = b->pass_tmp.as<int32_t>(); }
    EPI_TRY(epi_batch_threshold_reads_dev(b, thr.cls[0], thr.cls[1], thr.cls[2] ? thr.cls[2] : "", thr.cls[3] ? thr.cls[3] : "",
                                          thr.prm.min_n_ctx, thr.prm.min_ctx_meth_frac, thr.prm.max_ooctx_meth_frac, dst, s));
    *d_pass = dst;
  }
  return EPI_OK;
}

static uint32_t &cx_slot_state(epi_batch *b, uint32_t ctx_mask) { return (ctx_mask & ~(1u << 7)) ? b->cx_slot_wide : b->cx_slot_cg; }

static int cx_layout_pool(epi_batch *b, uint32_t ctx_mask, CxPlan &p) {
  uint32_t &slot_state = cx_slot_state(b, ctx_mask);
  if (!slot_state) slot_state = (ctx_mask & ~(1u << 7)) ? (uint32_t)(3 * p.T) / 4 : (uint32_t)p.T / 8;
  EPI_TRY(layout_pool(b, slot_state, p.T, p.nt, p.headroom, options().cx_slot, ensure_pool, &p.pool));
  b->cx_last_slot = p.pool.slot;
  b->cx_last_ovf = (uint32_t)p.pool.ovf_base;
  return EPI_OK;
}

static void cx_bind_pool(const epi_batch *b, Cx2Args &a) {
  a.tiles = b->tiles.as<Tile>();
  a.cursor = &report_scalars(b)->cursor;
  a.tile_nrow = b->tile_nrow.as<uint32_t>();
  a.tile_base = b->tile_base.as<uint32_t>();
  a.slab = b->d_slab;
  a.pool_key = b->pool_key.as<uint32_t>();
  a.pool_meth = b->pool_a.as<uint32_t>();
  a.pool_unmeth = b->pool_b.as<uint32_t>();
  a.pool_cap = (uint32_t)(b->pool_cap > 0xFFFFFFF0ull ? 0xFFFFFFF0ull : b->pool_cap);
  a.slot_rows = b->cx_last_slot;
  a.ovf_base = b->cx_last_ovf;
}

static int cx_fill_args(epi_batch *b, const CxPlan &p, const int32_t *d_pass, hipStream_t s, Cx2Args &a) {
  Scalars *sc = report_scalars(b);
  a.c.xm = b->xm; a.c.off = b->off; a.c.len = b->len; a.c.start = b->start; a.c.strand = b->strand; a.c.pass = p.fused ? nullptr : d_pass;
  a.xm_cap = (b->nbytes + 15) / 16 * 16;
  cx_bind_pool(b, a);
  a.heavy_rows = 16384;
  if (options().heavy_rows > 0) a.heavy_rows = options().heavy_rows;
  if (a.heavy_rows > 16384) a.heavy_rows = 16384;
  a.heavy_chunk = a.heavy_rows / 4 > 64 ? a.heavy_rows / 4 : 64;
  if (a.heavy_chunk > 256) a.heavy_chunk = 256;
  EPI_TRY(b->heavy_list.ensure((size_t)p.nt * 4));
  a.heavy_list = b->heavy_list.as<uint32_t>();
  a.heavy_count = &sc->heavy_count;
  a.heavy_max = &sc->heavy_max;
  a.heavy_slab = nullptr;
  if (p.per_tile) {
    EPI_TRY(b->deep_list.ensure((size_t)p.nt * 4));
    a.deep_list = b->deep_list.as<uint32_t>();
    a.deep_count = &sc->deep_count;
  }
  a.nrows = b->n;
#ifdef EPI_CHECK
  EPI_TRY(b->diag.ensure(256));
  a.dbg = b->diag.as<uint32_t>();
  EPI_HIP(hipMemsetAsync(a.dbg, 0, 32, s));
#endif
  return EPI_OK;
}

static int cx_queue_attempt(epi_batch *b, const CxPlan &p, Cx2Args &a, hipStream_t s, bool rezero) {
  if (rezero) {
    Scalars *sc = report_scalars(b);
    EPI_HIP(hipMemsetAsync(&sc->cursor, 0, offsetof(Scalars, fold_cursor) - offsetof(Scalars, cursor), s));
    EPI_HIP(hipMemsetAsync(&sc->heavy_max, 0, 4, s));
  }
  prof_begin("cx_tiles", s);
  launch_cx(false, p.np, p.fused, p.lean, p.shape, p.nt, dim3(1), s, a);
  prof_end("cx_tiles", s);
  if (p.per_tile) {
    Cx2Args g = a;
    g.tile_list = a.deep_list;
    g.tile_list_count = a.deep_count;
    g.deep_list = nullptr; g.deep_count = nullptr;
    prof_begin("cx_deep", s);
    launch_cx(false, p.np, p.fused, false, p.shape_heavy, p.nt, dim3(1), s, g);
    prof_end("cx_deep", s);
  }
  if (p.chained) {
    EPI_TRY(b->heavy_slab.ensure((size_t)CX_HEAVY_CAP * kCxPlanes * p.T * 4));
    a.heavy_slab = b->heavy_slab.as<int32_t>();
    a.heavy_first = 0;
    EPI_HIP(hipMemsetAsync(a.heavy_slab, 0, (size_t)CX_HEAVY_CAP * kCxPlanes * p.T * 4, s));
    prof_begin("cx_heavy", s);
    launch_cx(true, p.np, p.fused, p.lean, p.shape_heavy, p.nt, dim3(CX_HEAVY_GRID, CX_HEAVY_CAP), s, a);
    prof_end("cx_heavy", s);
  }
  EPI_HIP(hipGetLastError());
  return EPI_OK;
}

static int cx_finish_pool_run(epi_batch *b, const CxPlan &p, Cx2Args &a, hipStream_t s, int attempt, Scalars *host, bool *host_heavy) {
  Scalars *sc = report_scalars(b);
  EPI_TRY(scan_exclusive_u32(a.tile_nrow, b->tile_out.as<uint32_t>(), p.nt, &sc->rows, b->scan_tmp, s));
  EPI_TRY(read_report_scalars(b, s, host));
  EPI_TRY(cx_check_tile_count(b, p.nt_hinted, host->ntiles, p.nt));
  const uint32_t heavy_done = p.chained ? CX_HEAVY_CAP : 0u;
  if (host->heavy_count > heavy_done) {
    *host_heavy = true;
    b->cx_noheavy_T = 0;
    const uint32_t nheavy = host->heavy_count - heavy_done, nchunks = (host->heavy_max + (uint32_t)a.heavy_chunk - 1) / (uint32_t)a.heavy_chunk;
    a.heavy_first = (int)heavy_done;
    EPI_TRY(b->heavy_slab.ensure((size_t)nheavy * kCxPlanes * p.T * 4));
    a.heavy_slab = b->heavy_slab.as<int32_t>();
    EPI_HIP(hipMemsetAsync(a.heavy_slab, 0, (size_t)nheavy * kCxPlanes * p.T * 4, s));
    prof_begin("cx_heavy", s);
    launch_cx(true, p.np, p.fused, p.lean, p.shape_heavy, p.nt, dim3(nchunks, nheavy), s, a);
    prof_end("cx_heavy", s);
    EPI_HIP(hipGetLastError());
    EPI_TRY(scan_exclusive_u32(a.tile_nrow, b->tile_out.as<uint32_t>(), p.nt, &sc->rows, b->scan_tmp, s));
    EPI_TRY(read_report_scalars(b, s, host));
  }
#ifdef EPI_CHECK
  {
    uint32_t d[8];
    EPI_HIP(hipMemcpy(d, a.dbg, 32, hipMemcpyDeviceToHost));
    if (d[0]) return fail(EPI_ERR_STATE, "CX index check %u failed: v0=%lld v1=%d block=%u thread=%u (n=%lld nt=%d attempt=%d)", d[0],
                          (long long)(((uint64_t)d[5] << 32) | d[1]), (int)d[2], d[3], d[4], (long long)b->n, p.nt, attempt);
  }
#endif
  (void)attempt;
  return EPI_OK;
}

static int cx_keep_offsets(epi_batch *b, uint32_t ctx_mask, const CxPlan &p, uint32_t nrow, hipStream_t s) {
  if (b->cx_prev_key == (ctx_mask | 0x80000000u) && b->cx_prev_T == p.T && b->cx_prev_nt == p.nt) return EPI_OK;
  EPI_TRY(b->cx_prev_off.ensure((size_t)p.nt * 4));
  EPI_TRY(b->cx_prev_cnt.ensure((size_t)p.nt * 4));
  EPI_HIP(hipMemcpyAsync(b->cx_prev_off.p, b->tile_out.p, (size_t)p.nt * 4, hipMemcpyDeviceToDevice, s));
  EPI_HIP(hipMemcpyAsync(b->cx_prev_cnt.p, b->tile_nrow.p, (size_t)p.nt * 4, hipMemcpyDeviceToDevice, s));
  b->cx_prev_key = ctx_mask | 0x80000000u;
  b->cx_prev_T = p.T;
  b->cx_prev_nt = p.nt;
  b->cx_prev_nrow = nrow;
  return EPI_OK;
}

static int cx_report_impl(epi_batch *b, const int32_t *d_pass, const CxThreshold *thr, int32_t *d_pass_out, const char *ctx,
                          hipStream_t s, int64_t *nrow_out, int32_t *const *d_cols = nullptr, int64_t cap = 0,
                          int *written = nullptr) {
  *nrow_out = 0;
  if (written) *written = 0;
  b->last_kind = KIND_NONE;
  const uint32_t ctx_mask = ctx_mask_of(ctx);

  Cx2Args a;
  memset(&a, 0, sizeof(a));
  CxPlan p = {};
  p.np = make_report_lut(ctx_mask, &a.lut_r, &a.ctx_of_plane);
  a.lut_rx = lut16_xor_form(a.lut_r);
  a.fill4 = 0x0C0C0C0Cu;
  p.T = cx_tile_for(p.np);
  RowStats st;
  EPI_TRY(build_tiles(b, s, p.T, &st, &p.nt, &p.nt_hinted));
  b->last_ntiles = p.nt;
  if (thr) EPI_TRY(cx_setup_threshold(b, *thr, st, p, d_pass_out, s, a, &d_pass));
  if (p.nt == 0 || p.np == 0) {
    b->last_kind = !b->shared_keys.empty() && b->d_slab ? KIND_CX_SHARED : KIND_CX; b->last_nrow = 0; b->last_ntiles = 0;
    return EPI_OK;
  }
  const int T = p.T, np = p.np;
  const int32_t nt = p.nt;

  EPI_TRY(b->tile_nrow.ensure((size_t)nt * 4));
  EPI_TRY(b->tile_base.ensure((size_t)nt * 4));
  EPI_TRY(b->tile_out.ensure((size_t)(nt + 1) * 4));
  p.nshared = (int32_t)b->shared_keys.size();
  p.headroom = p.nshared > 0 ? (size_t)p.nshared * 2 * T : 0;
  EPI_TRY(cx_layout_pool(b, ctx_mask, p));
  p.lean = np == 1 && options().cx_lean;
  p.per_tile = p.lean && st.deep != 0;
  p.chained = st.deep != 0;
  p.shape = np > 1 ? pick_cxp_group(st) * 8 : pick_cx_shape(st, T, p.fused, p.lean);
  p.shape_heavy = np > 1 ? p.shape : pick_cx_shape(st, T, p.fused, false);
  b->cx_last_np = np;
  b->cx_last_ctx_of_plane = a.ctx_of_plane;
  EPI_TRY(check_grid(((int64_t)nt + 7) / 8 * 8, np == 1 && p.lean ? cx2_wg<true>() : CX_WG, "CX tile kernel"));
  EPI_TRY(cx_fill_args(b, p, d_pass, s, a));
  b->cx_deferred = false;

  const int64_t rec = cx_recorded_nrow(b, ctx_mask);
  bool direct = d_cols && cap > 0 && cap <= 0x7FFFFFFF && rec >= 0 && rec <= cap && st.deep == 0 && p.nshared == 0 && options().cx_direct &&
                b->cx_prev_T == T && b->cx_prev_nt == nt;
  for (int i = 0; direct && i < 6; i++) if (!d_cols[i]) direct = false;
  if (direct) {
    Cx2Args d = a;
    d.prev_off = b->cx_prev_off.as<uint32_t>();
    d.prev_nrow = b->cx_prev_cnt.as<uint32_t>();
    d.mismatch = d.cursor;
    for (int i = 0; i < 6; i++) d.out[i] = d_cols[i];
    d.out_cap = cap;
    d.heavy_rows = 0x7FFFFFFF;
    EPI_TRY(cx_queue_attempt(b, p, d, s, false));
    Scalars host;
    EPI_TRY(read_report_scalars(b, s, &host));
    EPI_TRY(cx_check_tile_count(b, p.nt_hinted, host.ntiles, nt));
    if (host.cursor == 0) {
      b->last_kind = KIND_NONE;
      b->last_nrow = 0;
      *nrow_out = b->cx_prev_nrow;
      if (written) *written = 1;
      return EPI_OK;
    }
    b->cx_prev_key = 0;
  }

  Scalars host;
  bool host_heavy = false;
  for (int run = 0;; run++) {
    cx_bind_pool(b, a);
    EPI_TRY(cx_queue_attempt(b, p, a, s, direct || run > 0));
    if (run == 0 && b->cx_defer && p.nshared > 0 && p.nt_hinted && b->cx_noheavy_T == T && b->cx_noheavy_rows == a.heavy_rows) {
      b->cx_deferred = true;
      b->cx_def_heavy_done = p.chained ? CX_HEAVY_CAP : 0u;
      b->last_kind = KIND_CX_SHARED;
      return EPI_OK;
    }
    EPI_TRY(cx_finish_pool_run(b, p, a, s, run + (direct ? 1 : 0), &host, &host_heavy));
    if (p.pool.ovf_base + host.cursor + p.headroom <= a.pool_cap) break;
    if (run == 1) return fail(EPI_ERR_STATE, "row pool overflow after regrow");
    EPI_TRY(ensure_pool(b, p.pool.ovf_base + host.cursor + (host.cursor >> 4) + 1024 + p.headroom));
    if (p.nshared > 0)
      EPI_HIP(hipMemsetAsync(b->d_slab, 0, (size_t)p.nshared * kCxPlanes * T * 4, s));
  }
  uint32_t &slot_state = cx_slot_state(b, ctx_mask);
  if (host.cursor > host.rows / 8 && slot_state < (uint32_t)(2 * T)) slot_state *= 2;
  if (!host_heavy) { b->cx_noheavy_T = T; b->cx_noheavy_rows = a.heavy_rows; }
  if (p.nshared > 0) { b->last_kind = KIND_CX_SHARED; return EPI_OK; }
  b->last_kind = KIND_CX;
  b->last_nrow = host.rows;
  *nrow_out = host.rows;
  return cx_keep_offsets(b, ctx_mask, p, host.rows, s);
}

}

using namespace epi;

extern "C" {

int epi_tile_positions(void) { return cx_tile_for(1); }

int epi_cx_tile_positions(const char *ctx) {
  uint32_t cop = 0;
  ClassLut l;
  return cx_tile_for(make_report_lut(ctx ? ctx_mask_of(ctx) : 0u, &l, &cop));
}

int epi_batch_cx_report_dev(epi_batch *b, const int32_t *d_pass, const char *ctx, void *stream, int64_t *nrow_out) {
  if (!b || !ctx || !nrow_out) return fail(EPI_ERR_ARG, "epi_batch_cx_report_dev: NULL argument");
  EPI_HIP(hipSetDevice(b->eng->device));
  return cx_report_impl(b, d_pass, nullptr, nullptr, ctx, pick_stream(b, stream), nrow_out);
}

int epi_batch_cytosine_report_dev(epi_batch *b, const char *ctx_meth, const char *ctx_unmeth, const char *ooctx_meth,
                                  const char *ooctx_unmeth, uint32_t min_n_ctx, double min_ctx_meth_frac,
                                  double max_ooctx_meth_frac, const char *ctx, int32_t *d_pass_out, void *stream,
                                  int64_t *nrow_out) {
  return epi_batch_cytosine_report_into_dev(b, ctx_meth, ctx_unmeth, ooctx_meth, ooctx_unmeth, min_n_ctx, min_ctx_meth_frac,
                                            max_ooctx_meth_frac, ctx, d_pass_out, nullptr, 0, stream, nrow_out, nullptr);
}

int epi_batch_cx_report_capacity(epi_batch *b, const char *ctx, int64_t *nrow) {
  if (!b || !ctx || !nrow) return fail(EPI_ERR_ARG, "epi_batch_cx_report_capacity: NULL argument");
  *nrow = cx_recorded_nrow(b, ctx_mask_of(ctx));
  return EPI_OK;
}

int epi_batch_cx_report_into_dev(epi_batch *b, const int32_t *d_pass, const char *ctx, int32_t *const d_cols[6], int64_t cap,
                                 void *stream, int64_t *nrow_out, int *written) {
  if (!b || !ctx || !nrow_out || !written || cap < 0 || (cap > 0 && !d_cols))
    return fail(EPI_ERR_ARG, "epi_batch_cx_report_into_dev: bad arguments");
  EPI_HIP(hipSetDevice(b->eng->device));
  return cx_report_impl(b, d_pass, nullptr, nullptr, ctx, pick_stream(b, stream), nrow_out, d_cols, cap, written);
}

int epi_batch_cytosine_report_into_dev(epi_batch *b, const char *ctx_meth, const char *ctx_unmeth, const char *ooctx_meth,
                                       const char *ooctx_unmeth, uint32_t min_n_ctx, double min_ctx_meth_frac,
                                       double max_ooctx_meth_frac, const char *ctx, int32_t *d_pass_out,
                                       int32_t *const d_cols[6], int64_t cap, void *stream, int64_t *nrow_out, int *written) {
  if (!b || !ctx || !nrow_out || !ctx_meth || !ctx_unmeth || cap < 0 || (cap > 0 && !d_cols))
    return fail(EPI_ERR_ARG, "epi_batch_cytosine_report_dev: bad arguments");
  EPI_HIP(hipSetDevice(b->eng->device));
  CxThreshold t;
  t.cls[0] = ctx_meth; t.cls[1] = ctx_unmeth; t.cls[2] = ooctx_meth ? ooctx_meth : ""; t.cls[3] = ooctx_unmeth ? ooctx_unmeth : "";
  t.prm.min_n_ctx = min_n_ctx; t.prm.min_ctx_meth_frac = min_ctx_meth_frac; t.prm.max_ooctx_meth_frac = max_ooctx_meth_frac;
  return cx_report_impl(b, nullptr, &t, d_pass_out, ctx, pick_stream(b, stream), nrow_out, d_cols, cap, written);
}

int epi_batch_cx_finish_shared(epi_batch *b, const char *ctx, void *stream, int64_t *nrow_out) {
  if (!b || !ctx || !nrow_out) return fail(EPI_ERR_ARG, "epi_batch_cx_finish_shared: NULL argument");
  if (b->last_kind != KIND_CX_SHARED) return fail(EPI_ERR_STATE, "epi_batch_cx_finish_shared without a sharded epi_batch_cx_report_dev");
  EPI_HIP(hipSetDevice(b->eng->device));
  hipStream_t s = pick_stream(b, stream);
  const int32_t nt = b->last_ntiles;
  if (nt == 0) { b->last_kind = KIND_CX; b->last_nrow = 0; *nrow_out = 0; return EPI_OK; }
  Cx2Args a;
  memset(&a, 0, sizeof(a));
  cx_bind_pool(b, a);
  a.ctx_of_plane = b->cx_last_ctx_of_plane;
  launch_cx_emit_slab(b->cx_last_np, (int)b->shared_keys.size(), s, a, b->d_shared_owned.as<int32_t>(),
                      b->d_slot_tile.as<int32_t>());
  EPI_HIP(hipGetLastError());
  EPI_TRY(scan_exclusive_u32(a.tile_nrow, b->tile_out.as<uint32_t>(), nt, &report_scalars(b)->rows, b->scan_tmp, s));
  Scalars host;
  EPI_TRY(read_report_scalars(b, s, &host));
  if (b->cx_deferred) {
    b->cx_deferred = false;
    EPI_TRY(cx_check_tile_count(b, true, host.ntiles, nt));
    if (host.heavy_count > b->cx_def_heavy_done) {
      b->cx_noheavy_T = 0;
      return fail(EPI_ERR_STATE, "ultra-deep tiles appeared in a batch that had none (%u): the rows of this batch changed", host.heavy_count);
    }
    if ((size_t)a.ovf_base + host.cursor > a.pool_cap) {
      b->last_kind = KIND_NONE;
      return EPI_RETRY_POOL;
    }
  }
  if ((size_t)a.ovf_base + host.cursor > a.pool_cap) return fail(EPI_ERR_STATE, "row pool overflow in sharded report");
  const uint32_t total = host.rows;
  b->last_kind = KIND_CX;
  b->last_nrow = total;
  *nrow_out = total;
  return EPI_OK;
}

int epi_batch_cx_set_shared(epi_batch *b, const int64_t *h_keys, const int32_t *h_owned, int32_t nshared,
                            int32_t *d_slab) {
  if (!b || nshared < 0 || (nshared > 0 && (!h_keys || !h_owned || !d_slab)))
    return fail(EPI_ERR_ARG, "epi_batch_cx_set_shared: bad arguments");
  for (int32_t i = 1; i < nshared; i++)
    if (h_keys[i - 1] >= h_keys[i]) return fail(EPI_ERR_ARG, "epi_batch_cx_set_shared: keys must be strictly increasing");
  EPI_HIP(hipSetDevice(b->eng->device));
  b->shared_keys.assign(h_keys, h_keys + nshared);
  b->shared_owned.assign(h_owned, h_owned + nshared);
  if (nshared > 0 && b->dev_shared_keys == b->shared_keys && b->dev_shared_owned == b->shared_owned) {
    b->d_slab = d_slab;
    b->d_mhl_cnt_slab = nullptr;
    b->d_mhl_sum_slab = nullptr;
    return EPI_OK;
  }
  b->d_slab = nshared > 0 ? d_slab : nullptr;
  b->d_mhl_cnt_slab = nullptr;
  b->d_mhl_sum_slab = nullptr;
  if (nshared > 0) {
    EPI_TRY(b->d_shared_keys.ensure((size_t)nshared * 8));
    EPI_TRY(b->d_shared_owned.ensure((size_t)nshared * 4));
    EPI_HIP(hipMemcpy(b->d_shared_keys.p, h_keys, (size_t)nshared * 8, hipMemcpyHostToDevice));
    EPI_HIP(hipMemcpy(b->d_shared_owned.p, h_owned, (size_t)nshared * 4, hipMemcpyHostToDevice));
    b->dev_shared_keys = b->shared_keys;
    b->dev_shared_owned = b->shared_owned;
  }
  return EPI_OK;
}

int epi_batch_tile_key_range(epi_batch *b, void *stream, int64_t *first_key, int64_t *last_key) {
  return epi_batch_tile_key_range_for(b, cx_tile_for(1), stream, first_key, last_key);
}

int epi_batch_tile_key_range_for(epi_batch *b, int tile_positions, void *stream, int64_t *first_key, int64_t *last_key) {
  if (!b || !first_key || !last_key) return fail(EPI_ERR_ARG, "epi_batch_tile_key_range: NULL argument");
  EPI_HIP(hipSetDevice(b->eng->device));
  hipStream_t s = pick_stream(b, stream);
  *first_key = 0; *last_key = -1;
  const int T = tile_positions;
  RowStats st;
  int32_t nt = 0;
  EPI_TRY(build_tiles(b, s, T, &st, &nt));
  if (nt == 0) return EPI_OK;
  Tile t0, t1;
  EPI_TRY(read_scalars(b, s, b->tiles.as<Tile>(), sizeof(Tile), &t0));
  EPI_TRY(read_scalars(b, s, b->tiles.as<Tile>() + (nt - 1), sizeof(Tile), &t1));
  auto key = [T](const Tile &t) { return ((int64_t)t.rname << 32) | (int64_t)(uint32_t)((t.pos0 + kPosBias) / T); };
  *first_key = key(t0);
  *last_key = key(t1);
  return EPI_OK;
}

int epi_batch_cx_fetch_dev(epi_batch *b, int32_t *const d_cols[6], void *stream) {
  if (!b || !d_cols) return fail(EPI_ERR_ARG, "epi_batch_cx_fetch_dev: NULL argument");
  if (b->last_kind != KIND_CX) return fail(EPI_ERR_STATE, "epi_batch_cx_fetch_dev: no finished CX report on this batch");
  if (b->last_nrow == 0) return EPI_OK;
  for (int i = 0; i < 6; i++) if (!d_cols[i]) return fail(EPI_ERR_ARG, "epi_batch_cx_fetch_dev: NULL column");
  EPI_HIP(hipSetDevice(b->eng->device));
  hipStream_t s = pick_stream(b, stream);
  const unsigned nb = (unsigned)((b->last_ntiles + 3) / 4);
  prof_begin("gather", s);
  hipLaunchKernelGGL(k_cx_gather, dim3(nb), dim3(256), 0, s, b->tiles.as<Tile>(), b->tile_out.as<uint32_t>(),
                     b->tile_nrow.as<uint32_t>(), b->tile_base.as<uint32_t>(), b->last_ntiles, b->pool_key.as<uint32_t>(),
                     b->pool_a.as<uint32_t>(), b->pool_b.as<uint32_t>(), d_cols[0], d_cols[1], d_cols[2], d_cols[3],
                     d_cols[4], d_cols[5]);
  prof_end("gather", s);
  EPI_HIP(hipGetLastError());
  return EPI_OK;
}

int epi_batch_cx_fetch_host(epi_batch *b, int32_t *const h_cols[6], void *stream) {
  if (!b || !h_cols) return fail(EPI_ERR_ARG, "epi_batch_cx_fetch_host: NULL argument");
  if (b->last_kind != KIND_CX) return fail(EPI_ERR_STATE, "epi_batch_cx_fetch_host: no finished CX report on this batch");
  const int64_t nrow = b->last_nrow;
  if (nrow == 0) return EPI_OK;
  EPI_HIP(hipSetDevice(b->eng->device));
  hipStream_t s = pick_stream(b, stream);
  EPI_TRY(b->pool_c.ensure((size_t)nrow * 4 * 6));
  int32_t *d = b->pool_c.as<int32_t>();
  int32_t *cols[6];
  for (int i = 0; i < 6; i++) cols[i] = d + (int64_t)i * nrow;
  EPI_TRY(epi_batch_cx_fetch_dev(b, cols, s));
  CopyPart parts[6];
  for (int i = 0; i < 6; i++) parts[i] = {h_cols[i], cols[i], (size_t)nrow * 4};
  return copy_parts_to_host(b->eng, parts, 6, s);
}

}
```

### epialleler_amd/csrc/engine.hip

```cpp
#include "common.hpp"
#include <algorithm>
#include <sys/mman.h>
#include <stdarg.h>
#include <stdio.h>
#include <stdlib.h>
#include <string.h>
#include <condition_variable>
#include <mutex>
#include <thread>
#include <vector>

namespace epi {

int DevBuf::ensure(size_t bytes) {
  if (bytes <= cap && p) return EPI_OK;
  if (bytes == 0) bytes = 16;
  size_t want = bytes + (bytes >> 3) + 256;
  if (p) { (void)hipFree(p); p = nullptr; cap = 0; }
  EPI_HIP(hipMalloc(&p, want));
  cap = want;
  return EPI_OK;
}

void DevBuf::release() {
  if (p) (void)hipFree(p);
  p = nullptr;
  cap = 0;
}

hipStream_t pick_stream(epi_batch *b, void *stream) {
  (void)b;
  return reinterpret_cast<hipStream_t>(stream);
}

int read_scalars(epi_batch *b, hipStream_t s, const void *d_src, size_t bytes, void *h_dst) {
  if (bytes > 512) return fail(EPI_ERR_ARG, "read_scalars: too large");
  EPI_HIP(hipMemcpyAsync(b->eng->h_scalars, d_src, bytes, hipMemcpyDeviceToHost, s));
  EPI_HIP(hipStreamSynchronize(s));
  memcpy(h_dst, b->eng->h_scalars, bytes);
  return EPI_OK;
}

static bool g_prof_on = false;
static std::mutex g_prof_mu;
struct Pending { std::string name; hipEvent_t a, b; };
static std::vector<Pending> g_pending;
static std::map<std::string, ProfEntry> g_prof;
static std::map<std::string, hipEvent_t> g_open;

void prof_begin(const char *name, hipStream_t s) {
  if (!g_prof_on) return;
  std::lock_guard<std::mutex> lk(g_prof_mu);
  hipEvent_t e;
  if (hipEventCreate(&e) != hipSuccess) return;
  (void)hipEventRecord(e, s);
  g_open[name] = e;
}

void prof_end(const char *name, hipStream_t s) {
  if (!g_prof_on) return;
  std::lock_guard<std::mutex> lk(g_prof_mu);
  auto it = g_open.find(name);
  if (it == g_open.end()) return;
  hipEvent_t e;
  if (hipEventCreate(&e) != hipSuccess) return;
  (void)hipEventRecord(e, s);
  g_pending.push_back({name, it->second, e});
  g_open.erase(it);
}

static void prof_drain() {
  for (auto &p : g_pending) {
    float ms = 0;
    if (hipEventSynchronize(p.b) == hipSuccess && hipEventElapsedTime(&ms, p.a, p.b) == hipSuccess) {
      g_prof[p.name].ms += ms;
      g_prof[p.name].n += 1;
    }
    (void)hipEventDestroy(p.a);
    (void)hipEventDestroy(p.b);
  }
  g_pending.clear();
}

}

using namespace epi;

extern "C" {

int epi_version(void) { return 100; }

void epi_prof_enable(int on) { g_prof_on = on != 0; }

int epi_prof_get(const char *name, double *ms_total, int64_t *launches) {
  std::lock_guard<std::mutex> lk(g_prof_mu);
  prof_drain();
  auto it = g_prof.find(name);
  if (it == g_prof.end()) { if (ms_total) *ms_total = 0; if (launches) *launches = 0; return EPI_OK; }
  if (ms_total) *ms_total = it->second.ms;
  if (launches) *launches = it->second.n;
  return EPI_OK;
}

void epi_prof_reset(void) {
  std::lock_guard<std::mutex> lk(g_prof_mu);
  prof_drain();
  g_prof.clear();
}

int epi_engine_create(int device, epi_engine **out) {
  if (!out) return fail(EPI_ERR_ARG, "epi_engine_create: out is NULL");
  *out = nullptr;
  int ndev = 0;
  hipError_t e = hipGetDeviceCount(&ndev);
  if (e != hipSuccess || ndev <= 0)
    return fail(EPI_ERR_NODEVICE, "no HIP device available (%s); libepihip has no CPU fallback",
                e == hipSuccess ? "device count 0" : hipGetErrorName(e));
  if (device < 0 || device >= ndev) return fail(EPI_ERR_ARG, "device %d out of range [0,%d)", device, ndev);
  EPI_HIP(hipSetDevice(device));
  epi_engine *eng = new epi_engine();
  eng->device = device;
  EPI_HIP(hipStreamCreateWithFlags(&eng->stream, hipStreamNonBlocking));
  EPI_HIP(hipStreamCreateWithFlags(&eng->copy_stream, hipStreamNonBlocking));
  EPI_HIP(hipStreamCreateWithFlags(&eng->aux_stream, hipStreamNonBlocking));
  EPI_HIP(hipHostMalloc(reinterpret_cast<void **>(&eng->h_scalars), 512, hipHostMallocDefault));
  *out = eng;
  return EPI_OK;
}

void epi_engine_destroy(epi_engine *e) {
  if (!e) return;
  (void)hipSetDevice(e->device);
  for (int i = 0; i < 2; i++) {
    if (e->pinned[i]) (void)hipHostFree(e->pinned[i]);
    if (e->pinned_done[i]) (void)hipEventDestroy(e->pinned_done[i]);
  }
  for (int i = 0; i < 2; i++) {
    if (e->dev_stage[i]) (void)hipFree(e->dev_stage[i]);
    if (e->up_done[i]) (void)hipEventDestroy(e->up_done[i]);
    if (e->stage_free[i]) (void)hipEventDestroy(e->stage_free[i]);
  }
  if (e->h_scalars) (void)hipHostFree(e->h_scalars);
  if (e->aux_stream) (void)hipStreamDestroy(e->aux_stream);
  if (e->stream) (void)hipStreamDestroy(e->stream);
  if (e->copy_stream) (void)hipStreamDestroy(e->copy_stream);
  delete e;
}

int epi_engine_device(const epi_engine *e) { return e ? e->device : -1; }

namespace {
struct CopyPool {
  std::mutex mu;
  std::condition_variable cv_work, cv_done;
  std::vector<std::thread> workers;
  char *dst = nullptr;
  const char *src = nullptr;
  size_t len = 0, part = 0;
  unsigned parts = 0, next = 0, pending = 0;
  uint64_t epoch = 0;
  bool stop = false;

  void run_part(unsigned i) {
    const size_t o = part * i;
    if (o < len) memcpy(dst + o, src + o, o + part > len ? len - o : part);
  }
  void worker() {
    uint64_t seen = 0;
    std::unique_lock<std::mutex> lk(mu);
    for (;;) {
      cv_work.wait(lk, [&]() { return stop || (epoch != seen && next < parts); });
      if (stop) return;
      while (next < parts) {
        const unsigned i = next++;
        lk.unlock();
        run_part(i);
        lk.lock();
        if (--pending == 0) cv_done.notify_all();
      }
      seen = epoch;
    }
  }
  void copy(void *d, const void *s, size_t n, unsigned k) {
    std::unique_lock<std::mutex> lk(mu);
    while (workers.size() + 1 < k) workers.emplace_back([this]() { worker(); });
    dst = static_cast<char *>(d); src = static_cast<const char *>(s); len = n;
    part = ((n + k - 1) / k + 4095) & ~(size_t)4095;
    parts = k; next = 0; pending = k; epoch++;
    cv_work.notify_all();
    while (next < parts) {
      const unsigned i = next++;
      lk.unlock();
      run_part(i);
      lk.lock();
      --pending;
    }
    cv_done.wait(lk, [&]() { return pending == 0; });
  }
  ~CopyPool() {
    { std::lock_guard<std::mutex> lk(mu); stop = true; }
    cv_work.notify_all();
    for (auto &t : workers) t.join();
  }
};
}

static void parallel_memcpy(void *dst, const void *src, size_t len) {
  static const unsigned hw = std::thread::hardware_concurrency();
  const unsigned k = len < (2u << 20) ? 1u : (hw >= 16 ? 8u : hw >= 8 ? 4u : hw >= 4 ? 2u : 1u);
  if (k == 1) { memcpy(dst, src, len); return; }
  static CopyPool pool;
  static std::mutex one;
  std::lock_guard<std::mutex> g(one);
  pool.copy(dst, src, len, k);
}

static bool is_pinned_host(const void *h_src) {
  hipPointerAttribute_t at;
  memset(&at, 0, sizeof(at));
  if (hipPointerGetAttributes(&at, h_src) != hipSuccess) { (void)hipGetLastError(); return false; }
  return at.type == hipMemoryTypeHost;
}

static int staged_upload(epi_engine *eng, void *d_dst, const void *h_src, size_t bytes) {
  const size_t stage = 64u << 20;
  size_t chunk = stage;
  if (options().upload_piece > 0 && (size_t)options().upload_piece < stage) chunk = (size_t)options().upload_piece;
  if (bytes && is_pinned_host(h_src)) {
    EPI_HIP(hipMemcpyAsync(d_dst, h_src, bytes, hipMemcpyHostToDevice, eng->copy_stream));
    return EPI_OK;
  }
  if (!eng->pinned[0]) {
    for (int i = 0; i < 2; i++) {
      EPI_HIP(hipHostMalloc(&eng->pinned[i], stage, hipHostMallocDefault));
      EPI_HIP(hipEventCreateWithFlags(&eng->pinned_done[i], hipEventDisableTiming));
    }
    eng->pinned_bytes = stage;
  }
  for (int i = 0; i < 2; i++) EPI_HIP(hipEventSynchronize(eng->pinned_done[i]));
  size_t done = 0;
  int k = 0;
  while (done < bytes) {
    size_t len = bytes - done < chunk ? bytes - done : chunk;
    EPI_HIP(hipEventSynchronize(eng->pinned_done[k]));
    parallel_memcpy(eng->pinned[k], static_cast<const char *>(h_src) + done, len);
    EPI_HIP(hipMemcpyAsync(static_cast<char *>(d_dst) + done, eng->pinned[k], len, hipMemcpyHostToDevice, eng->copy_stream));
    EPI_HIP(hipEventRecord(eng->pinned_done[k], eng->copy_stream));
    done += len;
    k ^= 1;
  }
  return EPI_OK;
}

static int upload_rows_congruent(epi_engine *eng, const uint8_t *h_xm, const int64_t *h_off, int64_t n, int64_t nbytes,
                                 const int64_t *d_src_off, const int32_t *d_len, const int64_t *d_dst_off, uint8_t *arena) {
  const bool pinned_src = is_pinned_host(h_xm);
  size_t chunk = 64u << 20;
  if (pinned_src) {
    chunk = ((size_t)nbytes / 8 + ((1u << 20) - 1)) & ~(size_t)((1u << 20) - 1);
    if (chunk < (16u << 20)) chunk = 16u << 20;
    if (chunk > (256u << 20)) chunk = 256u << 20;
  }
  if (options().upload_piece > 0) {
    chunk = (size_t)options().upload_piece;
    if (!pinned_src && chunk > (64u << 20)) chunk = 64u << 20;
  }
  if (eng->dev_stage_bytes < chunk) {
    for (int i = 0; i < 2; i++) {
      if (eng->dev_stage[i]) { EPI_HIP(hipFree(eng->dev_stage[i])); eng->dev_stage[i] = nullptr; }
      EPI_HIP(hipMalloc(&eng->dev_stage[i], chunk));
    }
    eng->dev_stage_bytes = chunk;
  }
  for (int i = 0; i < 2; i++) {
    if (!eng->up_done[i]) EPI_HIP(hipEventCreateWithFlags(&eng->up_done[i], hipEventDisableTiming));
    if (!eng->stage_free[i]) EPI_HIP(hipEventCreateWithFlags(&eng->stage_free[i], hipEventDisableTiming));
  }
  if (!pinned_src && !eng->pinned[0]) {
    for (int i = 0; i < 2; i++) {
      EPI_HIP(hipHostMalloc(&eng->pinned[i], 64u << 20, hipHostMallocDefault));
      EPI_HIP(hipEventCreateWithFlags(&eng->pinned_done[i], hipEventDisableTiming));
    }
    eng->pinned_bytes = 64u << 20;
  }
  if (!pinned_src) for (int i = 0; i < 2; i++) EPI_HIP(hipEventSynchronize(eng->pinned_done[i]));
  const int g = layout_group(nbytes, n);
  int k = 0;
  for (int64_t c0 = 0; c0 < nbytes; k ^= 1) {
    const int64_t c1 = nbytes - c0 < (int64_t)chunk ? nbytes : c0 + (int64_t)chunk;
    const void *src = h_xm + c0;
    if (!pinned_src) {
      EPI_HIP(hipEventSynchronize(eng->pinned_done[k]));
      parallel_memcpy(eng->pinned[k], src, (size_t)(c1 - c0));
      src = eng->pinned[k];
    }
    EPI_HIP(hipStreamWaitEvent(eng->copy_stream, eng->stage_free[k], 0));
    EPI_HIP(hipMemcpyAsync(eng->dev_stage[k], src, (size_t)(c1 - c0), hipMemcpyHostToDevice, eng->copy_stream));
    if (!pinned_src) EPI_HIP(hipEventRecord(eng->pinned_done[k], eng->copy_stream));
    EPI_HIP(hipEventRecord(eng->up_done[k], eng->copy_stream));
    const int64_t ra = c0 == 0 ? 0 : (std::upper_bound(h_off + 1, h_off + n + 1, c0) - (h_off + 1));
    const int64_t rb = (std::upper_bound(h_off, h_off + n, c1) - h_off) - 1;
    EPI_HIP(hipStreamWaitEvent(eng->aux_stream, eng->up_done[k], 0));
    if (rb >= ra)
      EPI_TRY(layout_copy_range(static_cast<const uint8_t *>(eng->dev_stage[k]), c0, c1, d_src_off, d_len, d_dst_off, ra, rb - ra + 1, g, arena,
                                eng->aux_stream));
    EPI_HIP(hipEventRecord(eng->stage_free[k], eng->aux_stream));
    c0 = c1;
  }
  return EPI_OK;
}

}

namespace epi {

static int ensure_staging(epi_engine *eng) {
  const size_t chunk = 64u << 20;
  if (!eng->pinned[0]) {
    for (int i = 0; i < 2; i++) {
      EPI_HIP(hipHostMalloc(&eng->pinned[i], chunk, hipHostMallocDefault));
      EPI_HIP(hipEventCreateWithFlags(&eng->pinned_done[i], hipEventDisableTiming));
    }
    eng->pinned_bytes = chunk;
  }
  return EPI_OK;
}

int stage_buffer(epi_engine *eng, int k, uint8_t **buf, size_t *cap) {
  EPI_TRY(ensure_staging(eng));
  EPI_HIP(hipEventSynchronize(eng->pinned_done[k & 1]));
  *buf = static_cast<uint8_t *>(eng->pinned[k & 1]);
  *cap = eng->pinned_bytes;
  return EPI_OK;
}

int stage_send(epi_engine *eng, int k, void *d_dst, size_t bytes) {
  if (bytes) EPI_HIP(hipMemcpyAsync(d_dst, eng->pinned[k & 1], bytes, hipMemcpyHostToDevice, eng->copy_stream));
  EPI_HIP(hipEventRecord(eng->pinned_done[k & 1], eng->copy_stream));
  return EPI_OK;
}

static void advise_huge(void *p, size_t n) {
  if (n < (4u << 20) || options().no_hugepage) return;
  const uintptr_t two = (uintptr_t)2 << 20;
  const uintptr_t lo = (reinterpret_cast<uintptr_t>(p) + two - 1) & ~(two - 1), hi = (reinterpret_cast<uintptr_t>(p) + n) & ~(two - 1);
  if (hi > lo) (void)madvise(reinterpret_cast<void *>(lo), hi - lo, MADV_HUGEPAGE);
}

int copy_parts_to_host(epi_engine *eng, const CopyPart *parts, int nparts, hipStream_t s) {
  const size_t piece = 8u << 20;
  struct Pending { void *dst; size_t len; int buf; };
  Pending pend = {nullptr, 0, 0};
  bool have = false, staged = false;
  int k = 0;
  hipEvent_t ev[2] = {nullptr, nullptr};
  auto drain = [&]() -> int {
    if (!have) return EPI_OK;
    EPI_HIP(hipEventSynchronize(ev[pend.buf]));
    parallel_memcpy(pend.dst, eng->pinned[pend.buf], pend.len);
    have = false;
    return EPI_OK;
  };
  for (int i = 0; i < nparts; i++) {
    const CopyPart &p = parts[i];
    if (!p.bytes) continue;
    if (is_pinned_host(p.dst)) { EPI_HIP(hipMemcpyAsync(p.dst, p.src, p.bytes, hipMemcpyDeviceToHost, s)); continue; }
    advise_huge(p.dst, p.bytes);
    if (!staged) {
      EPI_TRY(ensure_staging(eng));
      for (int j = 0; j < 2; j++) EPI_HIP(hipEventCreateWithFlags(&ev[j], hipEventDisableTiming));
      staged = true;
    }
    for (size_t done = 0; done < p.bytes; done += piece) {
      const size_t len = p.bytes - done < piece ? p.bytes - done : piece;
      hipError_t e1 = hipMemcpyAsync(eng->pinned[k], static_cast<const char *>(p.src) + done, len, hipMemcpyDeviceToHost, s);
      hipError_t e2 = e1 == hipSuccess ? hipEventRecord(ev[k], s) : e1;
      int rc = drain();
      if (e2 != hipSuccess || rc != EPI_OK) {
        (void)hipStreamSynchronize(s);
        for (int j = 0; j < 2; j++) if (ev[j]) (void)hipEventDestroy(ev[j]);
        return rc != EPI_OK ? rc : fail(EPI_ERR_HIP, "device to host copy failed: %s", hipGetErrorName(e2));
      }
      pend = {static_cast<char *>(p.dst) + done, len, k};
      have = true;
      k ^= 1;
    }
  }
  int rc = drain();
  hipError_t e = hipStreamSynchronize(s);
  for (int j = 0; j < 2; j++) if (ev[j]) (void)hipEventDestroy(ev[j]);
  if (rc != EPI_OK) return rc;
  if (e != hipSuccess) return fail(EPI_ERR_HIP, "device to host copy failed: %s", hipGetErrorName(e));
  return EPI_OK;
}

int copy_to_host(epi_engine *eng, void *h_dst, const void *d_src, size_t bytes, hipStream_t s) {
  const CopyPart p = {h_dst, d_src, bytes};
  return copy_parts_to_host(eng, &p, 1, s);
}

}

extern "C" {

int epi_batch_upload(epi_engine *e, const uint8_t *xm, const int64_t *off, const int32_t *rname,
                     const int32_t *strand, const int32_t *start, int64_t n, epi_batch **out) {
  if (!e || !out) return fail(EPI_ERR_ARG, "epi_batch_upload: NULL engine/out");
  *out = nullptr;
  if (n < 0 || n > 0x7FFFFFF0LL) return fail(EPI_ERR_ARG, "epi_batch_upload: n=%lld out of range", (long long)n);
  if (!off) return fail(EPI_ERR_ARG, "epi_batch_upload: off is NULL");
  if (n > 0 && (!rname || !strand || !start)) return fail(EPI_ERR_ARG, "epi_batch_upload: NULL column");
  const int64_t nbytes = off[n] - off[0];
  if (off[0] != 0) return fail(EPI_ERR_ARG, "epi_batch_upload: off[0] must be 0");
  if (nbytes < 0 || (nbytes > 0 && !xm)) return fail(EPI_ERR_ARG, "epi_batch_upload: bad xm/off");
  EPI_HIP(hipSetDevice(e->device));
  epi_batch *b = new epi_batch();
  b->eng = e;
  b->n = n;
  b->nbytes = nbytes;
  b->owns = true;
  int rc = EPI_OK;
  const int modulus = (n > 0 && nbytes > 0) ? options().realign : 0;
  DevBuf new_off;
  do {
    if ((rc = b->own_off.ensure((size_t)(n + 1) * 8))) break;
    if ((rc = b->own_rname.ensure((size_t)n * 4 + 4))) break;
    if ((rc = b->own_strand.ensure((size_t)n * 4 + 4))) break;
    if ((rc = b->own_start.ensure((size_t)n * 4 + 4))) break;
    if ((rc = staged_upload(e, b->own_off.p, off, (size_t)(n + 1) * 8))) break;
    if (n) {
      if ((rc = staged_upload(e, b->own_rname.p, rname, (size_t)n * 4))) break;
      if ((rc = staged_upload(e, b->own_strand.p, strand, (size_t)n * 4))) break;
      if ((rc = staged_upload(e, b->own_start.p, start, (size_t)n * 4))) break;
    }
    b->off = b->own_off.as<int64_t>();
    b->rname = b->own_rname.as<int32_t>();
    b->strand = b->own_strand.as<int32_t>();
    b->start = b->own_start.as<int32_t>();
    if ((rc = launch_row_stats(b, e->copy_stream))) break;
    if (modulus) {
      unsigned long long h_end = 0;
      uint32_t head = 0;
      if ((rc = layout_offsets(b, modulus, e->copy_stream, &new_off, &h_end, &head))) break;
      const size_t cap = ((size_t)h_end + 15) / 16 * 16 + 64;
      if ((rc = b->own_xm.ensure(cap))) break;
      uint8_t *arena = b->own_xm.as<uint8_t>();
      if ((head && hipMemsetAsync(arena, 0xFB, head, e->aux_stream) != hipSuccess) ||
          hipMemsetAsync(arena + h_end, 0xFB, cap - (size_t)h_end, e->aux_stream) != hipSuccess) { rc = fail(EPI_ERR_HIP, "memset failed"); break; }
      if ((rc = upload_rows_congruent(e, xm, off, n, nbytes, b->off, b->len, new_off.as<int64_t>(), arena))) break;
      if (hipStreamSynchronize(e->copy_stream) != hipSuccess || hipStreamSynchronize(e->aux_stream) != hipSuccess) {
        rc = fail(EPI_ERR_HIP, "upload failed: %s", hipGetErrorName(hipGetLastError())); break;
      }
      std::swap(b->own_off, new_off);
      b->off = b->own_off.as<int64_t>();
      b->nbytes = (int64_t)h_end;
      b->congruent = modulus;
    } else {
      const size_t cap = ((size_t)nbytes + 15) / 16 * 16 + 64;
      if ((rc = b->own_xm.ensure(cap))) break;
      if (hipMemsetAsync(static_cast<char *>(b->own_xm.p) + nbytes, 0xFB, cap - nbytes, e->copy_stream) != hipSuccess) {
        rc = fail(EPI_ERR_HIP, "memset failed"); break;
      }
      if (nbytes && (rc = staged_upload(e, b->own_xm.p, xm, (size_t)nbytes))) break;
      if (hipStreamSynchronize(e->copy_stream) != hipSuccess) { rc = fail(EPI_ERR_HIP, "upload failed: %s", hipGetErrorName(hipGetLastError())); break; }
    }
  } while (0);
  new_off.release();
  if (rc) {
    (void)hipStreamSynchronize(e->copy_stream); (void)hipStreamSynchronize(e->aux_stream);
    epi_batch_free(b);
    return rc;
  }
  b->xm = b->own_xm.as<uint8_t>();
  b->cols_owned = true;
  *out = b;
  return EPI_OK;
}

int epi_batch_adopt(epi_engine *e, const uint8_t *d_xm, int64_t xm_capacity, int64_t nbytes,
                    const int64_t *d_off, const int32_t *d_rname, const int32_t *d_strand,
                    const int32_t *d_start, int64_t n, epi_batch **out) {
  if (!e || !out) return fail(EPI_ERR_ARG, "epi_batch_adopt: NULL engine/out");
  *out = nullptr;
  if (n < 0 || n > 0x7FFFFFF0LL) return fail(EPI_ERR_ARG, "epi_batch_adopt: n out of range");
  if (!d_off || (n > 0 && (!d_rname || !d_strand || !d_start))) return fail(EPI_ERR_ARG, "epi_batch_adopt: NULL column");
  if (nbytes < 0 || (nbytes > 0 && !d_xm)) return fail(EPI_ERR_ARG, "epi_batch_adopt: bad xm");
  if ((reinterpret_cast<uintptr_t>(d_xm) & 15) != 0) return fail(EPI_ERR_ARG, "epi_batch_adopt: d_xm must be 16-byte aligned");
  if (xm_capacity < (nbytes + 15) / 16 * 16)
    return fail(EPI_ERR_ARG, "epi_batch_adopt: xm_capacity %lld < nbytes rounded up to 16 (%lld)",
                (long long)xm_capacity, (long long)((nbytes + 15) / 16 * 16));
  epi_batch *b = new epi_batch();
  b->eng = e;
  b->n = n;
  b->nbytes = nbytes;
  b->owns = false;
  b->xm = d_xm;
  b->off = d_off;
  b->rname = d_rname;
  b->strand = d_strand;
  b->start = d_start;
  EPI_HIP(hipSetDevice(e->device));
  const int rc = launch_row_stats(b, nullptr);
  if (rc) { epi_batch_free(b); return rc; }
  *out = b;
  return EPI_OK;
}

void epi_batch_free(epi_batch *b) {
  if (!b) return;
  (void)hipSetDevice(b->eng->device);
  DevBuf *bufs[] = {&b->own_xm, &b->own_off, &b->own_len, &b->own_rname, &b->own_strand, &b->own_start, &b->stats,
                    &b->scan_tmp, &b->tiles, &b->tile_nrow, &b->tile_base,
                    &b->tile_out, &b->pool_key, &b->pool_a, &b->pool_b, &b->pool_c, &b->pool_d, &b->pool_e, &b->pool_f,
                    &b->misc, &b->mhl_m, &b->mhl_h, &b->mhl_blk, &b->mhl_cont, &b->mhl_cur, &b->d_shared_keys, &b->d_shared_owned, &b->heavy_list, &b->heavy_slab, &b->heavy_sums, &b->deep_list, &b->mhlf_fold_slab, &b->diag, &b->d_slot_tile, &b->pass_tmp, &b->thr_tab, &b->mhl_keep_tab, &b->host_io, &b->tile_bsum[0], &b->tile_bsum[1], &b->tile_bsum[2], &b->tile_bsum[3], &b->own_slab, &b->own_slab2, &b->tiles_nt_dev, &b->cx_prev_off, &b->cx_prev_cnt,
                    &b->het_cx, &b->het_rank, &b->het_flag, &b->het_key, &b->het_sctx, &b->het_counts, &b->het_out, &b->het_scal,
                    &b->link_back, &b->link_blen, &b->link_bmean, &b->link_bflag, &b->link_bout,
                    &b->cmp_cx, &b->cmp_counts_b};
  for (DevBuf *d : bufs) d->release();
  if (b->stats_done) (void)hipEventDestroy(b->stats_done);
  delete b;
}

int64_t epi_batch_nrows(const epi_batch *b) { return b ? b->n : -1; }

void epi_cx_table_free(epi_cx_table *t) {
  if (!t) return;
  epi::table_block_release(t->rname);
  memset(t, 0, sizeof(*t));
}

void epi_mhl_table_free(epi_mhl_table *t) {
  if (!t) return;
  epi::table_block_release(t->length);
  memset(t, 0, sizeof(*t));
}

}
```

### epialleler_amd/csrc/layout.hip

```cpp
#include "common.hpp"
#include <utility>

namespace epi {

constexpr int LY_ROWS = 1024;

__device__ __forceinline__ uint32_t ly_item(const int32_t *__restrict__ start, const int32_t *__restrict__ len, int64_t x, int64_t n,
                                            uint32_t am) {
  const uint32_t l = (uint32_t)len[x];
  const uint32_t pad = x + 1 < n ? ((uint32_t)start[x + 1] - ((uint32_t)start[x] + l)) & am : 0u;
  return l + pad;
}

__device__ __forceinline__ unsigned long long ly_wave_incl(unsigned long long v, int lane) {
#pragma unroll
  for (int d = 1; d < 64; d <<= 1) {
    const unsigned long long o = __shfl_up(v, d, 64);
    if (lane >= d) v += o;
  }
  return v;
}

__device__ __forceinline__ unsigned long long ly_block_excl(unsigned long long v, unsigned long long *total, unsigned long long *s_w ) {
  const int lane = threadIdx.x & 63, wave = threadIdx.x >> 6;
  const unsigned long long inc = ly_wave_incl(v, lane);
  __syncthreads();
  if (lane == 63) s_w[wave] = inc;
  __syncthreads();
  if (threadIdx.x == 0) {
    unsigned long long acc = 0;
    for (int w = 0; w < 4; w++) { const unsigned long long t = s_w[w]; s_w[w] = acc; acc += t; }
    s_w[4] = acc;
  }
  __syncthreads();
  *total = s_w[4];
  return s_w[wave] + inc - v;
}

__global__ __launch_bounds__(256) void k_ly_sums(const int32_t *__restrict__ start, const int32_t *__restrict__ len, int64_t n, uint32_t am,
                                                  unsigned long long *__restrict__ bsum) {
  __shared__ unsigned long long s_w[5];
  const int64_t x0 = (int64_t)blockIdx.x * LY_ROWS + (int64_t)threadIdx.x * 4;
  unsigned long long v = 0;
#pragma unroll
  for (int i = 0; i < 4; i++) if (x0 + i < n) v += ly_item(start, len, x0 + i, n, am);
  unsigned long long total;
  (void)ly_block_excl(v, &total, s_w);
  if (threadIdx.x == 0) bsum[blockIdx.x] = total;
}

__global__ __launch_bounds__(256) void k_ly_scan(unsigned long long *__restrict__ bsum, int64_t nb, unsigned long long first,
                                                  unsigned long long *__restrict__ d_end) {
  __shared__ unsigned long long s_w[5];
  unsigned long long carry = first;
  for (int64_t base = 0; base < nb; base += 256) {
    const int64_t i = base + threadIdx.x;
    const unsigned long long v = i < nb ? bsum[i] : 0ull;
    unsigned long long total;
    const unsigned long long ex = ly_block_excl(v, &total, s_w);
    if (i < nb) bsum[i] = carry + ex;
    carry += total;
  }
  if (threadIdx.x == 0) *d_end = carry;
}

__global__ __launch_bounds__(256) void k_ly_offsets(const int32_t *__restrict__ start, const int32_t *__restrict__ len, int64_t n, uint32_t am,
                                                     const unsigned long long *__restrict__ bsum, const unsigned long long *__restrict__ d_end,
                                                     int64_t *__restrict__ off_out) {
  __shared__ unsigned long long s_w[5];
  const int64_t x0 = (int64_t)blockIdx.x * LY_ROWS + (int64_t)threadIdx.x * 4;
  uint32_t it[4];
  unsigned long long v = 0;
#pragma unroll
  for (int i = 0; i < 4; i++) { it[i] = x0 + i < n ? ly_item(start, len, x0 + i, n, am) : 0u; v += it[i]; }
  unsigned long long total;
  unsigned long long o = bsum[blockIdx.x] + ly_block_excl(v, &total, s_w);
#pragma unroll
  for (int i = 0; i < 4; i++) {
    if (x0 + i < n) off_out[x0 + i] = (int64_t)o;
    o += it[i];
  }
  if (blockIdx.x == 0 && threadIdx.x == 0) off_out[n] = (int64_t)*d_end;
}

struct __attribute__((packed, aligned(1))) LyU4u { uint32_t x, y, z, w; };

template <int G>
__global__ __launch_bounds__(256) void k_ly_copy(const uint8_t *__restrict__ src, int64_t c0, int64_t c1, const int64_t *__restrict__ src_off,
                                                  const int32_t *__restrict__ len, const int64_t *__restrict__ dst_off, int64_t row_a,
                                                  int64_t nrows, uint8_t *__restrict__ dst) {
  const int sub = threadIdx.x & (G - 1);
  const int64_t k = ((int64_t)blockIdx.x * 256 + threadIdx.x) / G;
  if (k >= nrows) return;
  const int64_t x = row_a + k;
  const int64_t s = src_off[x], d = dst_off[x];
  const int64_t L = len[x], e = s + L;
  int64_t lo = c0 > s ? c0 - s : 0, hi = (c1 < e ? c1 : e) - s;
  if (hi > lo) {
    const uint8_t *sp = src + (s - c0) + lo;
    uint8_t *dp = dst + d + lo;
    const int64_t nby = hi - lo;
    int64_t h = (16 - ((d + lo) & 15)) & 15;
    if (h > nby) h = nby;
    for (int64_t i = sub; i < h; i += G) dp[i] = sp[i];
    const int64_t nfull = (nby - h) >> 4;
    for (int64_t q = sub; q < nfull; q += G) {
      const LyU4u v = *reinterpret_cast<const LyU4u *>(sp + h + (q << 4));
      *reinterpret_cast<uint4 *>(dp + h + (q << 4)) = make_uint4(v.x, v.y, v.z, v.w);
    }
    for (int64_t i = h + (nfull << 4) + sub; i < nby; i += G) dp[i] = sp[i];
  }
  if ((e > c0 && e <= c1) || (e == 0 && c0 == 0)) {
    const int64_t gap = dst_off[x + 1] - d - L;
    for (int64_t i = sub; i < gap; i += G) dst[d + L + i] = (uint8_t)0xFB;
  }
}

int layout_group(int64_t nbytes, int64_t n) {
  const int64_t mean = n > 0 ? nbytes / n : 0;
  int g = 8;
  while (g < 64 && (int64_t)g * 64 < mean) g <<= 1;
  return g;
}

int layout_copy_range(const uint8_t *src, int64_t c0, int64_t c1, const int64_t *src_off, const int32_t *len, const int64_t *dst_off,
                      int64_t row_a, int64_t nrows, int g, uint8_t *dst, hipStream_t s) {
  if (nrows <= 0) return EPI_OK;
  const unsigned blocks = (unsigned)((nrows * g + 255) / 256);
#define EPI_LY(GG) hipLaunchKernelGGL((k_ly_copy<GG>), dim3(blocks), dim3(256), 0, s, src, c0, c1, src_off, len, dst_off, row_a, nrows, dst)
  if (g == 8) EPI_LY(8); else if (g == 16) EPI_LY(16); else if (g == 32) EPI_LY(32); else EPI_LY(64);
#undef EPI_LY
  EPI_HIP(hipGetLastError());
  return EPI_OK;
}

int layout_offsets(epi_batch *b, int modulus, hipStream_t s, DevBuf *new_off, unsigned long long *h_end, uint32_t *head) {
  const int64_t n = b->n;
  const int64_t nb = (n + LY_ROWS - 1) / LY_ROWS;
  const uint32_t am = (uint32_t)modulus - 1u;
  DevBuf tmp;
  int rc = EPI_OK;
  do {
    if ((rc = tmp.ensure((size_t)(nb + 2) * 8))) break;
    if ((rc = new_off->ensure((size_t)(n + 1) * 8))) break;
    unsigned long long *bsum = tmp.as<unsigned long long>(), *d_end = bsum + nb;
    int32_t first_start = 0;
    if ((rc = read_scalars(b, s, b->start, 4, &first_start))) break;
    *head = (uint32_t)first_start & am;
    hipLaunchKernelGGL(k_ly_sums, dim3((unsigned)nb), dim3(256), 0, s, b->start, b->len, n, am, bsum);
    hipLaunchKernelGGL(k_ly_scan, dim3(1), dim3(256), 0, s, bsum, nb, (unsigned long long)*head, d_end);
    hipLaunchKernelGGL(k_ly_offsets, dim3((unsigned)nb), dim3(256), 0, s, b->start, b->len, n, am, bsum, d_end, new_off->as<int64_t>());
    if (hipGetLastError() != hipSuccess) { rc = fail(EPI_ERR_HIP, "layout: launch failed"); break; }
    if ((rc = read_scalars(b, s, d_end, 8, h_end))) break;
  } while (0);
  tmp.release();
  return rc;
}

int realign_batch(epi_batch *b, int modulus, hipStream_t s) {
  if (modulus != 4 && modulus != 8 && modulus != 16) return fail(EPI_ERR_ARG, "realign: modulus must be 4, 8 or 16");
  if (b->congruent == modulus || b->n == 0) { b->congruent = modulus; return EPI_OK; }
  if (!b->stats_queued || !b->len) return fail(EPI_ERR_STATE, "realign: the batch has no row lengths yet");
  if (b->last_kind != KIND_NONE) return fail(EPI_ERR_STATE, "epi_batch_realign: call it before the first report on the batch");
  EPI_HIP(hipStreamWaitEvent(s, b->stats_done, 0));
  DevBuf new_off, new_xm;
  int rc = EPI_OK;
  do {
    unsigned long long h_end = 0;
    uint32_t head = 0;
    if ((rc = layout_offsets(b, modulus, s, &new_off, &h_end, &head))) break;
    const size_t cap = ((size_t)h_end + 15) / 16 * 16 + 64;
    if ((rc = new_xm.ensure(cap))) break;
    uint8_t *dst = new_xm.as<uint8_t>();
    if (head && hipMemsetAsync(dst, 0xFB, head, s) != hipSuccess) { rc = fail(EPI_ERR_HIP, "realign: memset failed"); break; }
    if (hipMemsetAsync(dst + h_end, 0xFB, cap - (size_t)h_end, s) != hipSuccess) { rc = fail(EPI_ERR_HIP, "realign: memset failed"); break; }
    if ((rc = layout_copy_range(b->xm, 0, INT64_MAX, b->off, b->len, new_off.as<int64_t>(), 0, b->n, layout_group(b->nbytes, b->n), dst, s))) break;
    if (hipStreamSynchronize(s) != hipSuccess) { rc = fail(EPI_ERR_HIP, "realign: %s", hipGetErrorName(hipGetLastError())); break; }
    if (!b->owns) {
      const size_t cb = (size_t)b->n * 4;
      if ((rc = b->own_rname.ensure(cb + 4)) || (rc = b->own_strand.ensure(cb + 4)) || (rc = b->own_start.ensure(cb + 4))) break;
      if (hipMemcpyAsync(b->own_rname.p, b->rname, cb, hipMemcpyDeviceToDevice, s) != hipSuccess ||
          hipMemcpyAsync(b->own_strand.p, b->strand, cb, hipMemcpyDeviceToDevice, s) != hipSuccess ||
          hipMemcpyAsync(b->own_start.p, b->start, cb, hipMemcpyDeviceToDevice, s) != hipSuccess ||
          hipStreamSynchronize(s) != hipSuccess) { rc = fail(EPI_ERR_HIP, "realign: column copy failed"); break; }
      b->rname = b->own_rname.as<int32_t>();
      b->strand = b->own_strand.as<int32_t>();
      b->start = b->own_start.as<int32_t>();
      b->owns = true;
    }
    std::swap(b->own_xm, new_xm);
    std::swap(b->own_off, new_off);
    b->xm = b->own_xm.as<uint8_t>();
    b->off = b->own_off.as<int64_t>();
    b->nbytes = (int64_t)h_end;
    b->congruent = modulus;
    b->cols_owned = true;
  } while (0);
  new_off.release(); new_xm.release();
  return rc;
}

}

using namespace epi;

extern "C" int epi_batch_realign(epi_batch *b, void *stream) {
  if (!b) return fail(EPI_ERR_ARG, "epi_batch_realign: NULL batch");
  EPI_HIP(hipSetDevice(b->eng->device));
  const int m = options().realign;
  if (m == 0) return EPI_OK;
  return realign_batch(b, m, pick_stream(b, stream));
}

extern "C" int epi_batch_layout(const epi_batch *b) { return b ? b->congruent : -1; }

extern "C" int epi_batch_view(const epi_batch *b, const uint8_t **d_xm, const int64_t **d_off, const int32_t **d_len, int64_t *nbytes) {
  if (!b) return fail(EPI_ERR_ARG, "epi_batch_view: NULL batch");
  if (d_xm) *d_xm = b->xm;
  if (d_off) *d_off = b->off;
  if (d_len) *d_len = b->len;
  if (nbytes) *nbytes = b->nbytes;
  return EPI_OK;
}
```

Measured before the change: 12070.

## Pad owned xm buffers front and back so lean kernels skip the edge-load path

Batches that own their xm copy now get a 16-byte guard band before the data and pad-byte fill after it, and are flagged as padded. Lean CX tile kernels get a PAD template instance that drops the per-row edge test and the byte-wise bounds-checked load, always using the vector load. The emit phase is also reworked: each wave computes its scan prefix itself instead of waiting on a serial thread-0 pass plus an extra barrier, and the kept offset/nrow are loaded once per tile. This adds template instances and code size, and relies on the pad byte being counted as a non-context class.

```diff
diff --git a/epialleler_amd/csrc/common.hpp b/epialleler_amd/csrc/common.hpp
--- a/epialleler_amd/csrc/common.hpp
+++ b/epialleler_amd/csrc/common.hpp
@@ -138,6 +138,8 @@
 };
 }
 
+namespace epi { constexpr int64_t kXmPad = 16; constexpr int kXmPadByte = 0x0C; }
+
 struct epi_batch {
   epi_engine *eng = nullptr;
   int64_t n = 0, nbytes = 0;
@@ -149,6 +151,7 @@
   int congruent = 0;
   bool cols_owned = false;
   epi::DevBuf own_xm, own_off, own_len, own_rname, own_strand, own_start;
+  bool xm_padded = false;
 
   epi::DevBuf stats;
   bool stats_queued = false, stats_host = false;
diff --git a/epialleler_amd/csrc/cx_report.hip b/epialleler_amd/csrc/cx_report.hip
--- a/epialleler_amd/csrc/cx_report.hip
+++ b/epialleler_amd/csrc/cx_report.hip
@@ -27,6 +27,7 @@
 struct Cx2Args {
   RowCols c;
   int64_t xm_cap;
+  int64_t xm_front;
   const Tile *tiles;
   uint32_t fill4;
   ClassLut lut_r;
@@ -134,6 +135,11 @@
   tab[n] = least | (most << 16);
 }
 
+__device__ __forceinline__ int cx2_decide(uint32_t n_m, uint32_t n_u, uint32_t o_m, uint32_t o_u, const Cx2Args &a) {
+  if ((EPI_CX_ABLATE & 1024) && !a.thr_tab) return cx2_threshold(n_m, n_u, o_m, o_u, a.thr);
+  return cx2_threshold_tab(n_m, n_u, o_m, o_u, a.thr, a.thr_tab);
+}
+
 struct Cx2Row {
   const uint8_t *base;
   int32_t rel, len;
@@ -156,14 +162,17 @@
   m[0] = (uint32_t)a; m[1] = (uint32_t)(a >> 32); m[2] = (uint32_t)b; m[3] = (uint32_t)(b >> 32);
 }
 
-template <int T, int G, int NU, int NP, bool FUSED, int MODE = 0, class LT, class F>
+template <int T, int G, int NU, int NP, bool FUSED, int MODE = 0, bool PAD = false, class LT, class F>
 __device__ __forceinline__ void cx2_visit(const Cx2Args &a, Cx2Row &g, int32_t cs, int32_t cz, int sub, int rcur,
                                           const LT &L, F fetch_next, uint32_t *carry = nullptr) {
   constexpr int C = T / CX_CH, Q = LT::Q;
   const int32_t cb = cs + sub;
   const int32_t tl = cz - cb;
   uint32_t w[NU][4];
-  if (__builtin_expect(g.edge, 0)) {
+  constexpr bool NO_EDGE = PAD || (EPI_CX_ABLATE & 256) != 0;
+  bool edge = false;
+  if constexpr (!NO_EDGE) edge = g.edge;
+  if (__builtin_expect(edge, 0)) {
 #pragma unroll
     for (int u = 0; u < NU; u++) {
 #pragma unroll
@@ -188,7 +197,7 @@
       const int32_t uq = tl / G < NU - 1 ? tl / G : NU - 1;
       const int64_t a_lo = p - a.c.xm, a_hi = a_lo + (tl >= 0 ? CX_CH * (int64_t)(uq * G) + CX_CH : 0);
       (void)a_lo; (void)a_hi;
-      if (!EPI_DEV_CHECK(a.dbg, tl < 0 || (a_lo >= 0 && a_hi <= a.xm_cap), 21, a_lo, a_hi)) return;
+      if (!EPI_DEV_CHECK(a.dbg, tl < 0 || (a_lo >= -a.xm_front && a_hi <= a.xm_cap), 21, a_lo, a_hi)) return;
     }
     if (EPI_CX_ABLATE & 1) p = reinterpret_cast<const uint8_t *>(reinterpret_cast<uintptr_t>(p) & ~(uintptr_t)15);
 #pragma unroll
@@ -273,8 +282,7 @@
     if constexpr (MODE == 0) {
       const uint32_t s01 = cx2_group_sum<G>(cls[0] | (cls[1] << 16)), s23 = cx2_group_sum<G>(cls[2] | (cls[3] << 16));
       const uint32_t n_all = s01 & 0xFFFFu, n_m = s01 >> 16;
-      g.ps = a.thr_tab ? cx2_threshold_tab(n_m, n_all - n_m, s23 & 0xFFFFu, s23 >> 16, a.thr, a.thr_tab)
-                       : cx2_threshold(n_m, n_all - n_m, s23 & 0xFFFFu, s23 >> 16, a.thr);
+      g.ps = cx2_decide(n_m, n_all - n_m, s23 & 0xFFFFu, s23 >> 16, a);
       if (a.pass_out && sub == 0 && (uint32_t)g.rel < (uint32_t)T) a.pass_out[rcur] = g.ps;
     }
     const uint32_t pm = g.ps ? 0x01010101u : 0u;
@@ -369,7 +377,7 @@
   }
 }
 
-template <int T, int G, int NU, int NP, bool FUSED, int WG, class LT>
+template <int T, int G, int NU, int NP, bool FUSED, int WG, bool PAD = false, class LT>
 __device__ __forceinline__ void cx2_rows(const Cx2Args &a, const Tile &td, int row_lo, int row_hi, const LT &L) {
   constexpr int R = 64 / G, NW = WG / 64, C = T / CX_CH;
   const int lane = L.tid & 63, wave = L.tid >> 6;
@@ -392,31 +400,30 @@
       g.c0 = g.rel >> 4;
       g.clast = (g.rel + v.len - 1) >> 4;
       g.base = a.c.xm + (v.o - g.rel);
-      g.edge = v.o < CX_CH || v.o + v.len + CX_CH > a.xm_cap;
+      g.edge = !PAD && (v.o < CX_CH || v.o + v.len + CX_CH > a.xm_cap);
       g.sidx = v.sd - 1;
       g.ps = v.ps;
       if constexpr (FUSED) {
         if (__builtin_expect(__ballot(g.clast - g.c0 >= G * NU) == 0ull, 1)) {
-          cx2_visit<T, G, NU, NP, true>(a, g, g.c0, g.clast, sub, rcur, L, fetch_next);
+          cx2_visit<T, G, NU, NP, true, 0, PAD>(a, g, g.c0, g.clast, sub, rcur, L, fetch_next);
         } else {
           uint32_t cls[4] = {0, 0, 0, 0};
           for (int32_t cs = g.c0; __ballot(cs <= g.clast) != 0ull; cs += G * NU)
-            cx2_visit<T, G, NU, NP, true, 1>(a, g, cs, g.clast, sub, rcur, L, fetch_next, cls);
+            cx2_visit<T, G, NU, NP, true, 1, PAD>(a, g, cs, g.clast, sub, rcur, L, fetch_next, cls);
           const uint32_t s01 = cx2_group_sum<G>(cls[0] | (cls[1] << 16)), s23 = cx2_group_sum<G>(cls[2] | (cls[3] << 16));
           const uint32_t n_all = s01 & 0xFFFFu, n_m = s01 >> 16;
-          g.ps = a.thr_tab ? cx2_threshold_tab(n_m, n_all - n_m, s23 & 0xFFFFu, s23 >> 16, a.thr, a.thr_tab)
-                           : cx2_threshold(n_m, n_all - n_m, s23 & 0xFFFFu, s23 >> 16, a.thr);
+          g.ps = cx2_decide(n_m, n_all - n_m, s23 & 0xFFFFu, s23 >> 16, a);
           if (a.pass_out && sub == 0 && (uint32_t)g.rel < (uint32_t)T) a.pass_out[rcur] = g.ps;
           const int32_t ca = g.c0 > 0 ? g.c0 : 0, cz = g.clast < C - 1 ? g.clast : C - 1;
           for (int32_t cs = ca; __ballot(cs <= cz) != 0ull; cs += G * NU)
-            cx2_visit<T, G, NU, NP, true, 2>(a, g, cs, cz, sub, rcur, L, fetch_next);
+            cx2_visit<T, G, NU, NP, true, 2, PAD>(a, g, cs, cz, sub, rcur, L, fetch_next);
         }
       } else {
         const int32_t ca = g.c0 > 0 ? g.c0 : 0, cz = g.clast < C - 1 ? g.clast : C - 1;
         if (__builtin_expect(__ballot(cz - ca >= G * NU) == 0ull, 1)) {
-          cx2_visit<T, G, NU, NP, false>(a, g, ca, cz, sub, rcur, L, fetch_next);
+          cx2_visit<T, G, NU, NP, false, 0, PAD>(a, g, ca, cz, sub, rcur, L, fetch_next);
         } else {
-          for (int32_t cs = ca; __ballot(cs <= cz) != 0ull; cs += G * NU) cx2_visit<T, G, NU, NP, false>(a, g, cs, cz, sub, rcur, L, fetch_next);
+          for (int32_t cs = ca; __ballot(cs <= cz) != 0ull; cs += G * NU) cx2_visit<T, G, NU, NP, false, 0, PAD>(a, g, cs, cz, sub, rcur, L, fetch_next);
         }
       }
       if (sub == 0) {
@@ -476,8 +483,16 @@
   return a.ovf_base + o;
 }
 
-__device__ __forceinline__ void cx_direct_none(const Cx2Args &a, int tile, uint32_t tid = threadIdx.x) {
-  if (a.prev_off && tid == 0 && a.prev_nrow[tile] != 0u) atomicAdd(a.mismatch, 1u);
+struct CxKept { uint32_t off, nrow; };
+__device__ __forceinline__ CxKept cx_kept_of(const Cx2Args &a, int tile) {
+  CxKept k = {0u, 0u};
+  if (EPI_CX_ABLATE & 64) k.off = (uint32_t)tile * (uint32_t)(a.out_cap / gridDim.x);
+  else if (a.prev_off) { k.off = a.prev_off[tile]; k.nrow = a.prev_nrow[tile]; }
+  return k;
+}
+
+__device__ __forceinline__ void cx_direct_none(const Cx2Args &a, const CxKept &kept, uint32_t tid = threadIdx.x) {
+  if (a.prev_off && tid == 0 && kept.nrow != 0u && !(EPI_CX_ABLATE & 64)) atomicAdd(a.mismatch, 1u);
 }
 
 template <int T, int NP> struct CxSrcLds {
@@ -543,7 +558,8 @@
 }
 
 template <int T, int NP, int WG = CX_WG, class SRC>
-__device__ __forceinline__ void cx2_emit(const Cx2Args &a, int tile, const SRC &src, uint32_t *s_scan, uint16_t *s_list, uint32_t tid = threadIdx.x) {
+__device__ __forceinline__ void cx2_emit(const Cx2Args &a, int tile, const Tile &td, const CxKept &kept, const SRC &src, uint32_t *s_scan,
+                                         uint16_t *s_list, uint32_t tid = threadIdx.x) {
   constexpr int NW = WG / 64, PW = T / NW, IT = PW / 32;
   static_assert(PW % 32 == 0 && IT >= 1 && IT <= 16, "emit phase layout");
   const int lane = tid & 63, wave = tid >> 6;
@@ -594,30 +610,27 @@
   if (lane == 0) s_scan[wave] = carry;
   __syncthreads();
   if (a.prev_off) {
-    if (tid == 0) {
-      uint32_t acc = 0;
-      for (int w = 0; w < NW; w++) { const uint32_t t = s_scan[w]; s_scan[w] = acc; acc += t; }
-      const uint32_t base = a.prev_off[tile];
-      const bool good = acc == a.prev_nrow[tile] && (int64_t)base + acc <= a.out_cap;
-      if (!good) atomicAdd(a.mismatch, 1u);
-      s_scan[NW + 1] = good ? base : 0xFFFFFFFFu;
-    }
-    __syncthreads();
-    const uint32_t base = s_scan[NW + 1];
-    if (base != 0xFFFFFFFFu) {
-      const Tile td = a.tiles[tile];
-      const uint32_t w0 = base + s_scan[wave];
-#pragma unroll
-      for (int jj = 0; jj < IT; jj++) {
-        if (ok[jj]) {
-          const uint32_t o = w0 + off[jj];
+    uint32_t acc = 0, before = 0;
+#pragma unroll
+    for (int w = 0; w < NW; w++) { const uint32_t t = s_scan[w]; before += w < wave ? t : 0u; acc += t; }
+    const bool good = (acc == kept.nrow || (EPI_CX_ABLATE & 64)) && (int64_t)kept.off + acc <= a.out_cap;
+    if (!good) {
+      if (tid == 0 && !(EPI_CX_ABLATE & 64)) atomicAdd(a.mismatch, 1u);
+      return;
+    }
+    const uint32_t w0 = kept.off + before;
+#pragma unroll
+    for (int jj = 0; jj < IT; jj++) {
+      if (ok[jj]) {
+        const uint32_t o = w0 + off[jj];
+        if (!(EPI_CX_ABLATE & 128)) {
           a.out[0][o] = td.rname;
           a.out[1][o] = 1 + (int32_t)((key[jj] >> 3) & 1u);
-          a.out[2][o] = (int32_t)(td.pos0 + (int64_t)(key[jj] >> 4));
           a.out[3][o] = (int32_t)(key[jj] & 7u);
-          a.out[4][o] = (int32_t)me[jj];
-          a.out[5][o] = (int32_t)un[jj];
         }
+        a.out[2][o] = (int32_t)(td.pos0 + (int64_t)(key[jj] >> 4));
+        a.out[4][o] = (int32_t)me[jj];
+        a.out[5][o] = (int32_t)un[jj];
       }
     }
     return;
@@ -732,14 +745,14 @@
   for (int i = L.tid; i < LdsT::N_COV / 4; i += WG) x[i] = make_uint4(0, 0, 0, 0);
 }
 
-template <int T, int G, int NU, int NP, bool FUSED, bool LEAN, int WG>
+template <int T, int G, int NU, int NP, bool FUSED, bool LEAN, int WG, bool PAD = false>
 __device__ __forceinline__ void cx2_accumulate(const Cx2Args &a, const Tile &td, int row_lo, int row_hi, const Cx2Lds<T, NP, LEAN> &L) {
   if constexpr (LEAN) {
-    cx2_rows<T, G, NU, NP, FUSED, WG>(a, td, row_lo, row_hi, L);
+    cx2_rows<T, G, NU, NP, FUSED, WG, PAD>(a, td, row_lo, row_hi, L);
   } else {
     for (int b0 = row_lo; b0 < row_hi; b0 += CX_FLUSH_ROWS) {
       if (b0 > row_lo) { __syncthreads(); cx2_flush<T, NP, LEAN, WG>(L); __syncthreads(); }
-      cx2_rows<T, G, NU, NP, FUSED, WG>(a, td, b0, b0 + CX_FLUSH_ROWS < row_hi ? b0 + CX_FLUSH_ROWS : row_hi, L);
+      cx2_rows<T, G, NU, NP, FUSED, WG, PAD>(a, td, b0, b0 + CX_FLUSH_ROWS < row_hi ? b0 + CX_FLUSH_ROWS : row_hi, L);
     }
   }
   __syncthreads();
@@ -752,8 +765,8 @@
 #endif
 template <bool LEAN> constexpr int cx2_wg() { return LEAN ? EPI_CX_LEAN_WG : CX_WG; }
 
-template <int T, int G, int NU, int NP, bool FUSED, bool LEAN, class LdsT>
-__device__ __forceinline__ void cx2_tile(const Cx2Args &a, int tile, const Tile &td, const LdsT &L, uint32_t *s_scan, uint16_t *s_list, int *s_flag) {
+template <int T, int G, int NU, int NP, bool FUSED, bool LEAN, bool PAD = false, class LdsT>
+__device__ __forceinline__ void cx2_tile(const Cx2Args &a, int tile, const Tile &td, const CxKept &kept, const LdsT &L, uint32_t *s_scan, uint16_t *s_list, int *s_flag) {
   constexpr int WG = cx2_wg<LEAN>();
   cx2_clear<T, NP, LEAN, WG>(L);
   if (td.row_hi - td.row_lo > a.heavy_rows) {
@@ -764,7 +777,7 @@
       a.tile_nrow[tile] = 0;
       a.tile_base[tile] = 0;
     }
-    cx_direct_none(a, tile, L.tid);
+    cx_direct_none(a, kept, L.tid);
     return;
   }
   if constexpr (LEAN) {
@@ -778,35 +791,36 @@
       __syncthreads();
       if (*s_flag) {
         if (L.tid == 0) { a.deep_list[atomicAdd(a.deep_count, 1u)] = (uint32_t)tile; a.tile_nrow[tile] = 0; a.tile_base[tile] = 0; }
-        cx_direct_none(a, tile, L.tid);
+        cx_direct_none(a, kept, L.tid);
         return;
       }
     }
   }
   __syncthreads();
-  cx2_accumulate<T, G, NU, NP, FUSED, LEAN, WG>(a, td, td.row_lo, td.row_hi, L);
+  cx2_accumulate<T, G, NU, NP, FUSED, LEAN, WG, PAD>(a, td, td.row_lo, td.row_hi, L);
   if (td.slot >= 0) {
     cx2_dump_slab<T, NP, LEAN, WG>(L, a.slab + (int64_t)td.slot * (kCxPlanes * T));
     if (L.tid == 0) { a.tile_nrow[tile] = 0; a.tile_base[tile] = 0; }
-    cx_direct_none(a, tile, L.tid);
+    cx_direct_none(a, kept, L.tid);
     return;
   }
-  if (EPI_CX_ABLATE & 16) { if (L.tid == 0) { a.tile_nrow[tile] = 0; a.tile_base[tile] = 0; } cx_direct_none(a, tile, L.tid); return; }
+  if (EPI_CX_ABLATE & 16) { if (L.tid == 0) { a.tile_nrow[tile] = 0; a.tile_base[tile] = 0; } cx_direct_none(a, kept, L.tid); return; }
   cx2_prefix<T, WG>(L.cov, s_scan, L.tid);
   if constexpr (LEAN) {
     static_assert(NP == 1, "the u8 counters serve single-context reports");
     CxSrcU8<LdsT::Q> src;
     src.narrow = reinterpret_cast<const uint32_t *>(L.narrow); src.cov = L.cov;
-    cx2_emit<T, NP, WG>(a, tile, src, s_scan, s_list, L.tid);
+    cx2_emit<T, NP, WG>(a, tile, td, kept, src, s_scan, s_list, L.tid);
   } else {
     CxSrcLds<T, NP> src;
     src.wide = L.wide; src.cov = L.cov;
-    cx2_emit<T, NP, WG>(a, tile, src, s_scan, s_list, L.tid);
-  }
-}
-
-template <int T, int G, int NU, int NP, bool FUSED, bool LEAN>
+    cx2_emit<T, NP, WG>(a, tile, td, kept, src, s_scan, s_list, L.tid);
+  }
+}
+
+template <int T, int G, int NU, int NP, bool FUSED, bool LEAN, bool PAD = false>
 __global__ __launch_bounds__(cx2_wg<LEAN>(), (cx2_waves_per_simd<T, NP, NU, LEAN, cx2_wg<LEAN>()>())) void k_cx_tiles(Cx2Args a, int ntiles) {
+  static_assert(LEAN || !PAD, "the padded-batch instances exist for the lean kernels only");
   CX2_SHARED(T, NP, LEAN)
   __shared__ int s_flag;
   if constexpr (!LEAN) {
@@ -815,7 +829,8 @@
       for (uint32_t i = blockIdx.x; i < n; i += gridDim.x) {
         const int tile = (int)a.tile_list[i];
         const Tile td = a.tiles[tile];
-        cx2_tile<T, G, NU, NP, FUSED, LEAN>(a, tile, td, L, s_scan, s_list, &s_flag);
+        const CxKept kept = cx_kept_of(a, tile);
+        cx2_tile<T, G, NU, NP, FUSED, LEAN, PAD>(a, tile, td, kept, L, s_scan, s_list, &s_flag);
         __syncthreads();
       }
       return;
@@ -824,7 +839,8 @@
   const int tile = cx_tile_of_block(blockIdx.x, ntiles);
   if (tile >= ntiles) return;
   const Tile td = a.tiles[tile];
-  cx2_tile<T, G, NU, NP, FUSED, LEAN>(a, tile, td, L, s_scan, s_list, &s_flag);
+  const CxKept kept = cx_kept_of(a, tile);
+  cx2_tile<T, G, NU, NP, FUSED, LEAN, PAD>(a, tile, td, kept, L, s_scan, s_list, &s_flag);
 }
 
 template <int T, int G, int NU, int NP, bool FUSED>
@@ -856,7 +872,8 @@
   cx2_prefix<T>(s_cov + T, s_scan);
   CxSrcSlab<T, NP> src;
   src.slab = slab; src.cov = s_cov;
-  cx2_emit<T, NP>(a, tile, src, s_scan, s_list);
+  const Tile td = a.tiles[tile];
+  cx2_emit<T, NP>(a, tile, td, cx_kept_of(a, tile), src, s_scan, s_list);
 }
 
 template <int T, int NP>
@@ -992,26 +1009,27 @@
       a.tile_nrow[tile] = 0;
       a.tile_base[tile] = 0;
     }
-    cx_direct_none(a, tile);
+    cx_direct_none(a, cx_kept_of(a, tile));
     return;
   }
   __syncthreads();
   cxp_accumulate<G>(a.c, td, cnt);
+  const CxKept kept = cx_kept_of(a, tile);
   __syncthreads();
   cxp_convert(cnt);
   __syncthreads();
   if (td.slot >= 0) {
     cxp_dump_slab(a, cnt, np, a.slab + (int64_t)td.slot * (kCxPlanes * CXP_T));
     if (threadIdx.x == 0) { a.tile_nrow[tile] = 0; a.tile_base[tile] = 0; }
-    cx_direct_none(a, tile);
+    cx_direct_none(a, kept);
     return;
   }
   if (EPI_CX_ABLATE & 16) {
     if (threadIdx.x == 0) { a.tile_nrow[tile] = 0; a.tile_base[tile] = 0; }
-    cx_direct_none(a, tile);
+    cx_direct_none(a, kept);
     return;
   }
-  cx2_emit<CXP_T, 3>(a, tile, cxp_source(a, cnt), s_scan, s_list);
+  cx2_emit<CXP_T, 3>(a, tile, td, kept, cxp_source(a, cnt), s_scan, s_list);
 }
 
 template <int G>
@@ -1127,22 +1145,28 @@
 constexpr unsigned CX_HEAVY_CAP = 8, CX_HEAVY_GRID = 128;
 constexpr unsigned CX_LIST_GRID = 512;
 
-template <int T, int NU, int NP, bool FUSED, bool LEAN>
+template <int T, int NU, int NP, bool FUSED, bool LEAN, bool PAD = false>
 static void launch_cx_tiles(int g, int nt, hipStream_t s, const Cx2Args &a) {
   const unsigned nb = a.tile_list ? CX_LIST_GRID : (unsigned)(((nt + 7) / 8) * 8);
   switch (g) {
-    case 4: if constexpr (FUSED || LEAN) { hipLaunchKernelGGL((k_cx_tiles<T, 4, NU, NP, FUSED, LEAN>), dim3(nb), dim3(cx2_wg<LEAN>()), 0, s, a, nt); } break;
-    case 8: hipLaunchKernelGGL((k_cx_tiles<T, 8, NU, NP, FUSED, LEAN>), dim3(nb), dim3(cx2_wg<LEAN>()), 0, s, a, nt); break;
-    case 16: hipLaunchKernelGGL((k_cx_tiles<T, 16, NU, NP, FUSED, LEAN>), dim3(nb), dim3(cx2_wg<LEAN>()), 0, s, a, nt); break;
-    case 32: hipLaunchKernelGGL((k_cx_tiles<T, 32, NU, NP, FUSED, LEAN>), dim3(nb), dim3(cx2_wg<LEAN>()), 0, s, a, nt); break;
-    default: hipLaunchKernelGGL((k_cx_tiles<T, 64, NU, NP, FUSED, LEAN>), dim3(nb), dim3(cx2_wg<LEAN>()), 0, s, a, nt); break;
-  }
+    case 4: if constexpr (FUSED || LEAN) { hipLaunchKernelGGL((k_cx_tiles<T, 4, NU, NP, FUSED, LEAN, PAD>), dim3(nb), dim3(cx2_wg<LEAN>()), 0, s, a, nt); } break;
+    case 8: hipLaunchKernelGGL((k_cx_tiles<T, 8, NU, NP, FUSED, LEAN, PAD>), dim3(nb), dim3(cx2_wg<LEAN>()), 0, s, a, nt); break;
+    case 16: hipLaunchKernelGGL((k_cx_tiles<T, 16, NU, NP, FUSED, LEAN, PAD>), dim3(nb), dim3(cx2_wg<LEAN>()), 0, s, a, nt); break;
+    case 32: hipLaunchKernelGGL((k_cx_tiles<T, 32, NU, NP, FUSED, LEAN, PAD>), dim3(nb), dim3(cx2_wg<LEAN>()), 0, s, a, nt); break;
+    default: hipLaunchKernelGGL((k_cx_tiles<T, 64, NU, NP, FUSED, LEAN, PAD>), dim3(nb), dim3(cx2_wg<LEAN>()), 0, s, a, nt); break;
+  }
+}
+
+template <int T, int NU, int NP, bool FUSED>
+static void launch_cx_lean(int g, int nt, hipStream_t s, const Cx2Args &a) {
+  if (a.xm_front >= CX_CH && !(EPI_CX_ABLATE & 512)) launch_cx_tiles<T, NU, NP, FUSED, true, true>(g, nt, s, a);
+  else launch_cx_tiles<T, NU, NP, FUSED, true, false>(g, nt, s, a);
 }
 
 template <int T, int NU, int NP, bool FUSED>
 static void launch_cx_g(bool heavy, bool lean, int g, int nt, dim3 grid, hipStream_t s, const Cx2Args &a) {
   if (!heavy) {
-    if (lean) launch_cx_tiles<T, NU, NP, FUSED, true>(g, nt, s, a);
+    if (lean) launch_cx_lean<T, NU, NP, FUSED>(g, nt, s, a);
     else launch_cx_tiles<T, NU, NP, FUSED, false>(g, nt, s, a);
     return;
   }
@@ -1206,9 +1230,9 @@
   if (np > 1) { launch_cxp(heavy, np, g, nt, grid, s, a); return; }
   if (!heavy && lean && (shape & 7) > 3) {
     switch (shape & 7) {
-      case 4: if (fused) launch_cx_tiles<CX_T1, 4, 1, true, true>(g, nt, s, a); else launch_cx_tiles<CX_T1, 4, 1, false, true>(g, nt, s, a); break;
-      case 5: if (fused) launch_cx_tiles<CX_T1, 5, 1, true, true>(g, nt, s, a); else launch_cx_tiles<CX_T1, 5, 1, false, true>(g, nt, s, a); break;
-      default: if (fused) launch_cx_tiles<CX_T1, 6, 1, true, true>(g, nt, s, a); else launch_cx_tiles<CX_T1, 6, 1, false, true>(g, nt, s, a); break;
+      case 4: if (fused) launch_cx_lean<CX_T1, 4, 1, true>(g, nt, s, a); else launch_cx_lean<CX_T1, 4, 1, false>(g, nt, s, a); break;
+      case 5: if (fused) launch_cx_lean<CX_T1, 5, 1, true>(g, nt, s, a); else launch_cx_lean<CX_T1, 5, 1, false>(g, nt, s, a); break;
+      default: if (fused) launch_cx_lean<CX_T1, 6, 1, true>(g, nt, s, a); else launch_cx_lean<CX_T1, 6, 1, false>(g, nt, s, a); break;
     }
     return;
   }
@@ -1338,6 +1362,7 @@
       b->thr_tab_prm.max_ooctx_meth_frac = thr.prm.max_ooctx_meth_frac;
     }
     a.thr_tab = b->thr_tab.as<uint32_t>();
+    if (!a.thr_tab || b->thr_tab_len < st.max_len) return fail(EPI_ERR_STATE, "fused thresholding: the decision table covers %d < %d bytes", (int)b->thr_tab_len, (int)st.max_len);
   } else if (b->n > 0) {
     int32_t *dst = d_pass_out;
     if (!dst) { EPI_TRY(b->pass_tmp.ensure((size_t)b->n * 4)); dst = b->pass_tmp.as<int32_t>(); }
@@ -1376,7 +1401,10 @@
 static int cx_fill_args(epi_batch *b, const CxPlan &p, const int32_t *d_pass, hipStream_t s, Cx2Args &a) {
   Scalars *sc = report_scalars(b);
   a.c.xm = b->xm; a.c.off = b->off; a.c.len = b->len; a.c.start = b->start; a.c.strand = b->strand; a.c.pass = p.fused ? nullptr : d_pass;
-  a.xm_cap = (b->nbytes + 15) / 16 * 16;
+  a.xm_front = b->xm_padded ? kXmPad : 0;
+  a.xm_cap = (b->nbytes + 15) / 16 * 16 + (b->xm_padded ? kXmPad : 0);
+  static_assert(kXmPad >= CX_CH, "the pad holds a whole chunk");
+  if ((EPI_CX_ABLATE & 256) && !b->xm_padded) return fail(EPI_ERR_STATE, "timing build without the edge path: the batch must own a padded copy of xm");
   cx_bind_pool(b, a);
   a.heavy_rows = 16384;
   if (options().heavy_rows > 0) a.heavy_rows = options().heavy_rows;
diff --git a/epialleler_amd/csrc/engine.hip b/epialleler_amd/csrc/engine.hip
--- a/epialleler_amd/csrc/engine.hip
+++ b/epialleler_amd/csrc/engine.hip
@@ -443,10 +443,11 @@
       uint32_t head = 0;
       if ((rc = layout_offsets(b, modulus, e->copy_stream, &new_off, &h_end, &head))) break;
       const size_t cap = ((size_t)h_end + 15) / 16 * 16 + 64;
-      if ((rc = b->own_xm.ensure(cap))) break;
-      uint8_t *arena = b->own_xm.as<uint8_t>();
-      if ((head && hipMemsetAsync(arena, 0xFB, head, e->aux_stream) != hipSuccess) ||
-          hipMemsetAsync(arena + h_end, 0xFB, cap - (size_t)h_end, e->aux_stream) != hipSuccess) { rc = fail(EPI_ERR_HIP, "memset failed"); break; }
+      if ((rc = b->own_xm.ensure((size_t)kXmPad + cap))) break;
+      uint8_t *arena = b->own_xm.as<uint8_t>() + kXmPad;
+      if (hipMemsetAsync(arena - kXmPad, kXmPadByte, (size_t)kXmPad, e->aux_stream) != hipSuccess ||
+          (head && hipMemsetAsync(arena, 0xFB, head, e->aux_stream) != hipSuccess) ||
+          hipMemsetAsync(arena + h_end, kXmPadByte, cap - (size_t)h_end, e->aux_stream) != hipSuccess) { rc = fail(EPI_ERR_HIP, "memset failed"); break; }
       if ((rc = upload_rows_congruent(e, xm, off, n, nbytes, b->off, b->len, new_off.as<int64_t>(), arena))) break;
       if (hipStreamSynchronize(e->copy_stream) != hipSuccess || hipStreamSynchronize(e->aux_stream) != hipSuccess) {
         rc = fail(EPI_ERR_HIP, "upload failed: %s", hipGetErrorName(hipGetLastError())); break;
@@ -457,11 +458,13 @@
       b->congruent = modulus;
     } else {
       const size_t cap = ((size_t)nbytes + 15) / 16 * 16 + 64;
-      if ((rc = b->own_xm.ensure(cap))) break;
-      if (hipMemsetAsync(static_cast<char *>(b->own_xm.p) + nbytes, 0xFB, cap - nbytes, e->copy_stream) != hipSuccess) {
+      if ((rc = b->own_xm.ensure((size_t)kXmPad + cap))) break;
+      uint8_t *arena = b->own_xm.as<uint8_t>() + kXmPad;
+      if (hipMemsetAsync(arena - kXmPad, kXmPadByte, (size_t)kXmPad, e->copy_stream) != hipSuccess ||
+          hipMemsetAsync(arena + nbytes, kXmPadByte, cap - nbytes, e->copy_stream) != hipSuccess) {
         rc = fail(EPI_ERR_HIP, "memset failed"); break;
       }
-      if (nbytes && (rc = staged_upload(e, b->own_xm.p, xm, (size_t)nbytes))) break;
+      if (nbytes && (rc = staged_upload(e, arena, xm, (size_t)nbytes))) break;
       if (hipStreamSynchronize(e->copy_stream) != hipSuccess) { rc = fail(EPI_ERR_HIP, "upload failed: %s", hipGetErrorName(hipGetLastError())); break; }
     }
   } while (0);
@@ -471,7 +474,8 @@
     epi_batch_free(b);
     return rc;
   }
-  b->xm = b->own_xm.as<uint8_t>();
+  b->xm = b->own_xm.as<uint8_t>() + kXmPad;
+  b->xm_padded = true;
   b->cols_owned = true;
   *out = b;
   return EPI_OK;
diff --git a/epialleler_amd/csrc/layout.hip b/epialleler_amd/csrc/layout.hip
--- a/epialleler_amd/csrc/layout.hip
+++ b/epialleler_amd/csrc/layout.hip
@@ -170,10 +170,11 @@
     uint32_t head = 0;
     if ((rc = layout_offsets(b, modulus, s, &new_off, &h_end, &head))) break;
     const size_t cap = ((size_t)h_end + 15) / 16 * 16 + 64;
-    if ((rc = new_xm.ensure(cap))) break;
-    uint8_t *dst = new_xm.as<uint8_t>();
+    if ((rc = new_xm.ensure((size_t)kXmPad + cap))) break;
+    uint8_t *dst = new_xm.as<uint8_t>() + kXmPad;
+    if (hipMemsetAsync(dst - kXmPad, kXmPadByte, (size_t)kXmPad, s) != hipSuccess) { rc = fail(EPI_ERR_HIP, "realign: memset failed"); break; }
     if (head && hipMemsetAsync(dst, 0xFB, head, s) != hipSuccess) { rc = fail(EPI_ERR_HIP, "realign: memset failed"); break; }
-    if (hipMemsetAsync(dst + h_end, 0xFB, cap - (size_t)h_end, s) != hipSuccess) { rc = fail(EPI_ERR_HIP, "realign: memset failed"); break; }
+    if (hipMemsetAsync(dst + h_end, kXmPadByte, cap - (size_t)h_end, s) != hipSuccess) { rc = fail(EPI_ERR_HIP, "realign: memset failed"); break; }
     if ((rc = layout_copy_range(b->xm, 0, INT64_MAX, b->off, b->len, new_off.as<int64_t>(), 0, b->n, layout_group(b->nbytes, b->n), dst, s))) break;
     if (hipStreamSynchronize(s) != hipSuccess) { rc = fail(EPI_ERR_HIP, "realign: %s", hipGetErrorName(hipGetLastError())); break; }
     if (!b->owns) {
@@ -190,7 +191,8 @@
     }
     std::swap(b->own_xm, new_xm);
     std::swap(b->own_off, new_off);
-    b->xm = b->own_xm.as<uint8_t>();
+    b->xm = b->own_xm.as<uint8_t>() + kXmPad;
+    b->xm_padded = true;
     b->off = b->own_off.as<int64_t>();
     b->nbytes = (int64_t)h_end;
     b->congruent = modulus;
```

After: 11850. 1.9% lower.
